# AshishKumar4/FlaxDiff

Hardware: AMD Instinct MI355X
Metric: train images/sec/node (64x64 uncond EDM UNet, bs=256) (higher is better)
Workload: dtype bf16; 1 GPU; model=unet_64px_[64,128,256,512]_res2_heads4, global_batch=256, resolution=64, parallelism=dp1, schedule=EDM + KarrasPredictionTransform(sigma_data=0.5)

## Files before the change

flaxdiff_amd/models/common.py:

```python
from __future__ import annotations

import math
from typing import Callable, Optional

import torch
import torch.nn as nn
import torch.nn.functional as F

from .. import ops


_TRUNC_STD_CORRECTION = 0.87962566103423978


def variance_scaling_(tensor: torch.Tensor, fan_in: int, fan_out: int,
                      scale: float = 1.0, mode: str = "fan_in") -> torch.Tensor:
    if mode == "fan_in":
        denom = max(1, fan_in)
    elif mode == "fan_out":
        denom = max(1, fan_out)
    else:
        denom = max(1.0, (fan_in + fan_out) / 2)
    std = math.sqrt(max(scale, 1e-10) / denom) / _TRUNC_STD_CORRECTION
    with torch.no_grad():
        tensor.normal_(0.0, std)
        tensor.clamp_(-2 * std, 2 * std)
    return tensor


class _ShadowCast(torch.autograd.Function):

    @staticmethod
    def forward(ctx, p):
        return p._shadow_bf16

    @staticmethod
    def backward(ctx, dy):
        return dy.float()


def _cast(p: Optional[torch.Tensor], dtype) -> Optional[torch.Tensor]:
    if p is None:
        return None
    if p.dtype == dtype:
        return p
    if dtype == torch.bfloat16 and getattr(p, "_shadow_bf16", None) is not None:
        return _ShadowCast.apply(p)
    return p.to(dtype)



class Dense(nn.Module):
    def __init__(self, in_features: int, out_features: int, use_bias: bool = True,
                 kernel_scale: float = 1.0, zero_init: bool = False):
        super().__init__()
        self.in_features = in_features
        self.out_features = out_features
        w = torch.empty(in_features, out_features)
        if zero_init:
            nn.init.zeros_(w)
        else:
            variance_scaling_(w, in_features, out_features, scale=kernel_scale)
        self.weight = nn.Parameter(w)
        self.bias = nn.Parameter(torch.zeros(out_features)) if use_bias else None

    def forward(self, x: torch.Tensor, add: torch.Tensor = None) -> torch.Tensor:
        if x.is_cuda and x.dtype == torch.bfloat16:
            return ops.dense(x, self.weight, self.bias, add=add)
        return ops.dense(x, _cast(self.weight, x.dtype),
                         _cast(self.bias, x.dtype), add=add)



class GroupNorm(nn.Module):

    def __init__(self, num_groups: int, num_channels: int, eps: float = 1e-5):
        super().__init__()
        assert num_channels % num_groups == 0, (num_groups, num_channels)
        self.num_groups = num_groups
        self.eps = eps
        self.weight = nn.Parameter(torch.ones(num_channels))
        self.bias = nn.Parameter(torch.zeros(num_channels))

    def forward(self, x: torch.Tensor, silu: bool = False) -> torch.Tensor:
        if x.is_cuda:
            return ops.group_norm(x, self.num_groups, self.weight, self.bias,
                                  self.eps, silu)
        return ops.group_norm(x, self.num_groups, _cast(self.weight, x.dtype),
                              _cast(self.bias, x.dtype), self.eps, silu)


class RMSNorm(nn.Module):
    def __init__(self, dim: int, eps: float = 1e-5):
        super().__init__()
        self.eps = eps
        self.weight = nn.Parameter(torch.ones(dim))

    def forward(self, x: torch.Tensor) -> torch.Tensor:
        if x.is_cuda:
            return ops.rms_norm(x, self.weight, self.eps)
        return ops.rms_norm(x, _cast(self.weight, x.dtype), self.eps)



class TimeEmbedding(nn.Module):

    def __init__(self, features: int, max_positions: int = 10000):
        super().__init__()
        self.features = features
        self.max_positions = max_positions

    def forward(self, t: torch.Tensor) -> torch.Tensor:
        return ops.sinusoidal_time_embedding(t, self.features, self.max_positions)


class FourierEmbedding(nn.Module):

    def __init__(self, features: int, scale: float = 16.0):
        super().__init__()
        g = torch.Generator().manual_seed(42)
        freqs = torch.randn(features // 2, generator=g) * scale
        self.register_buffer("freqs", freqs, persistent=True)

    def forward(self, t: torch.Tensor) -> torch.Tensor:
        return ops.fourier_time_embedding(t, self.freqs)


class TimeProjection(nn.Module):

    def __init__(self, in_features: int, features: int):
        super().__init__()
        self.dense1 = Dense(in_features, features)
        self.dense2 = Dense(features, features)

    def forward(self, x: torch.Tensor) -> torch.Tensor:
        x = F.gelu(self.dense1(x))
        x = F.gelu(self.dense2(x))
        return x



class Conv(nn.Module):

    def __init__(self, in_features: int, features: int, kernel_size=(3, 3),
                 strides=(1, 1), use_bias: bool = True):
        super().__init__()
        kh, kw = kernel_size if isinstance(kernel_size, (tuple, list)) \
            else (kernel_size, kernel_size)
        self.stride = strides[0] if isinstance(strides, (tuple, list)) else strides
        w = torch.empty(kh, kw, in_features, features)
        variance_scaling_(w, kh * kw * in_features, kh * kw * features)
        self.weight = nn.Parameter(w)
        self.bias = nn.Parameter(torch.zeros(features)) if use_bias else None

    def forward(self, x: torch.Tensor, add: torch.Tensor = None,
                badd: torch.Tensor = None) -> torch.Tensor:
        if x.is_cuda and x.dtype == torch.bfloat16:
            return ops.conv2d(x, self.weight, self.bias, stride=self.stride,
                              add=add, badd=badd)
        return ops.conv2d(x, _cast(self.weight, x.dtype), _cast(self.bias, x.dtype),
                          stride=self.stride, add=add, badd=badd)


class ConvTranspose(nn.Module):
    def __init__(self, in_features: int, features: int, kernel_size=(3, 3), strides=(2, 2)):
        super().__init__()
        kh, kw = kernel_size
        self.stride = strides[0]
        w = torch.empty(kh, kw, in_features, features)
        variance_scaling_(w, kh * kw * in_features, kh * kw * features)
        self.weight = nn.Parameter(w)
        self.bias = nn.Parameter(torch.zeros(features))

    def forward(self, x):
        return ops.conv2d_transpose(x, _cast(self.weight, x.dtype),
                                    _cast(self.bias, x.dtype), stride=self.stride)


class SeparableConv(nn.Module):

    def __init__(self, in_features: int, features: int, kernel_size=(3, 3),
                 strides=(1, 1), use_bias: bool = False):
        super().__init__()
        kh, kw = kernel_size
        self.stride = strides[0] if isinstance(strides, (tuple, list)) else strides
        dw = torch.empty(kh, kw, in_features, 1)
        variance_scaling_(dw, kh * kw, kh * kw)
        self.depthwise = nn.Parameter(dw)
        pw = torch.empty(1, 1, in_features, features)
        variance_scaling_(pw, in_features, features)
        self.pointwise = nn.Parameter(pw)
        self.bias = nn.Parameter(torch.zeros(features)) if use_bias else None

    def forward(self, x):
        x = ops.depthwise_conv2d(x, _cast(self.depthwise, x.dtype), None, self.stride)
        return ops.conv2d(x, _cast(self.pointwise, x.dtype), _cast(self.bias, x.dtype), 1)


class WeightStandardizedConv(nn.Module):

    def __init__(self, in_features: int, features: int, kernel_size=(3, 3), strides=(1, 1)):
        super().__init__()
        kh, kw = kernel_size
        self.stride = strides[0] if isinstance(strides, (tuple, list)) else strides
        w = torch.empty(kh, kw, in_features, features)
        variance_scaling_(w, kh * kw * in_features, kh * kw * features)
        self.weight = nn.Parameter(w)
        self.bias = nn.Parameter(torch.zeros(features))

    def forward(self, x):
        w = self.weight
        eps = 1e-5 if x.dtype == torch.float32 else 1e-3
        mean = w.mean(dim=(0, 1, 2), keepdim=True)
        var = w.var(dim=(0, 1, 2), unbiased=False, keepdim=True)
        w = (w - mean) / torch.sqrt(var + eps)
        return ops.conv2d(x, _cast(w, x.dtype), _cast(self.bias, x.dtype), self.stride)


def ConvLayer(conv_type: str, in_features: int, features: int, kernel_size=(3, 3),
              strides=(1, 1)) -> nn.Module:
    if conv_type == "conv":
        return Conv(in_features, features, kernel_size, strides)
    if conv_type == "w_conv":
        return WeightStandardizedConv(in_features, features, kernel_size, strides)
    if conv_type == "separable":
        return SeparableConv(in_features, features, kernel_size, strides)
    if conv_type == "conv_transpose":
        return ConvTranspose(in_features, features, kernel_size, strides)
    raise ValueError(f"unknown conv_type {conv_type}")


class PixelShuffle(nn.Module):

    def __init__(self, scale: int):
        super().__init__()
        self.scale = scale

    def forward(self, x):
        B, H, W, C = x.shape
        s = self.scale
        c = C // (s * s)
        x = x.reshape(B, H, W, s, s, c)
        x = x.permute(0, 1, 3, 2, 4, 5)
        return x.reshape(B, H * s, W * s, c)


class Upsample(nn.Module):

    def __init__(self, in_features: int, features: int, scale: int = 2,
                 activation: Callable = F.silu):
        super().__init__()
        assert scale == 2
        self.conv = Conv(in_features, features, (3, 3), (1, 1))

    def forward(self, x, residual=None):
        if x.is_cuda and x.dtype == torch.bfloat16:
            out = ops.conv2d_upsample2x(x, self.conv.weight, self.conv.bias)
        else:
            out = self.conv(ops.nearest_upsample_2x(x))
        if residual is not None:
            out = ops.cat_channels(out, residual)
        return out


class Downsample(nn.Module):

    def __init__(self, in_features: int, features: int, scale: int = 2,
                 activation: Callable = F.silu):
        super().__init__()
        assert scale == 2
        self.conv = Conv(in_features, features, (3, 3), (2, 2))

    def forward(self, x, residual=None):
        out = self.conv(x)
        if residual is not None:
            if residual.shape[1] > out.shape[1]:
                residual = ops.avg_pool_2x(residual)
            out = ops.cat_channels(out, residual)
        return out



class ResidualBlock(nn.Module):

    def __init__(self, conv_type: str, in_features: int, features: int,
                 temb_features: int, kernel_size=(3, 3), strides=(1, 1),
                 activation: Callable = F.silu, norm_groups: int = 8,
                 norm_epsilon: float = 1e-4):
        super().__init__()
        self.features = features
        self.activation = activation
        self._fused_silu = activation in (F.silu, torch.nn.functional.silu)
        if norm_groups > 0:
            self.norm1 = GroupNorm(norm_groups, in_features, eps=norm_epsilon)
            self.norm2 = GroupNorm(norm_groups, features, eps=norm_epsilon)
        else:
            self.norm1 = RMSNorm(in_features, eps=norm_epsilon)
            self.norm2 = RMSNorm(features, eps=norm_epsilon)
        self.conv1 = ConvLayer(conv_type, in_features, features, kernel_size, strides)
        self.temb_projection = Dense(temb_features, features)
        self.conv2 = ConvLayer(conv_type, features, features, kernel_size, strides)
        self.residual_conv = (ConvLayer(conv_type, in_features, features, (1, 1), (1, 1))
                              if in_features != features else None)

    def _norm_act(self, norm, x):
        if isinstance(norm, GroupNorm) and self._fused_silu:
            return norm(x, silu=True)
        return self.activation(norm(x))

    def forward(self, x: torch.Tensor, temb: torch.Tensor,
                textemb: torch.Tensor = None, extra_features: torch.Tensor = None):
        residual = x
        out = self._norm_act(self.norm1, x)
        t = self.temb_projection(temb.to(out.dtype))
        if isinstance(self.conv1, Conv):
            out = self.conv1(out, badd=t)
        else:
            out = self.conv1(out) + t[:, None, None, :]

        out = self._norm_act(self.norm2, out)
        if self.residual_conv is not None:
            residual = self.residual_conv(residual)
        if isinstance(self.conv2, Conv) and residual.shape[-1] == self.features:
            out = self.conv2(out, add=residual)
        else:
            out = self.conv2(out) + residual

        if extra_features is not None:
            out = ops.cat_channels(out, extra_features)
        return out


def l2norm(t: torch.Tensor, dim=1, eps=1e-6):
    return t / torch.clamp(t.norm(p=2, dim=dim, keepdim=True), min=eps)
```

flaxdiff_amd/ops/__init__.py:

```python
from __future__ import annotations

import os
import weakref
from typing import Optional

import torch

from . import reference

_EXT = None
_EXT_ERR: Optional[str] = None


def _load_ext():
    global _EXT, _EXT_ERR
    if _EXT is not None or _EXT_ERR is not None:
        return _EXT
    try:
        from .hip import build as hip_build
        _EXT = hip_build.load_extension()
    except Exception as e:
        _EXT_ERR = f"{type(e).__name__}: {e}"
        _EXT = None
    return _EXT


def hip_available() -> bool:
    return _load_ext() is not None


def _require_ext():
    ext = _load_ext()
    if ext is None:
        raise RuntimeError(
            "flaxdiff_amd HIP extension is not available on a GPU tensor path "
            f"(build error: {_EXT_ERR}). Run __graft_entry__.build() / "
            "python -m flaxdiff_amd.ops.hip.build first — the GPU path never "
            "silently falls back to stock torch ops.")
    return ext


_FORCE_TORCH = os.environ.get("FLAXDIFF_FORCE_TORCH_OPS", "0") == "1"
_GEMM_LIB = os.environ.get("FD_GEMM_LIB", "0") == "1"


def _use_hip(x: torch.Tensor) -> bool:
    return x.is_cuda and not _FORCE_TORCH



_GRAD_HOOK_OWNERS: "weakref.WeakSet" = weakref.WeakSet()


def register_grad_hook_owner(owner) -> None:
    _GRAD_HOOK_OWNERS.add(owner)


def _sink_kinds() -> str:
    v = os.environ.get("FD_GRAD_SINK", "1")
    if v == "0":
        return ""
    return "wbgr" if v == "all" else "bgr"


def grad_sinks_active() -> bool:
    if not _sink_kinds():
        return False
    return not any(o.hooks_live for o in _GRAD_HOOK_OWNERS)


def _grad_sink(p: Optional[torch.Tensor], kind: str) -> Optional[torch.Tensor]:
    if p is None or kind not in _sink_kinds():
        return None
    sink = getattr(p, "_grad_sink", None)
    if sink is None or sink.dtype != torch.float32 or not grad_sinks_active():
        return None
    owner = getattr(p, "_grad_sink_owner", None)
    g = (p if owner is None else owner).grad
    if g is None or g.data_ptr() != sink.data_ptr() \
            or g.numel() != sink.numel() or not sink.is_contiguous():
        return None
    return sink



class _GroupNormSiLUFn(torch.autograd.Function):
    @staticmethod
    def forward(ctx, x, gamma, beta, groups, eps, silu):
        ext = _require_ext()
        y, mean, rstd = ext.gn_silu_fwd(x, gamma, beta, groups, eps, silu)
        ctx.save_for_backward(x, gamma, mean, rstd)
        ctx.groups = groups
        ctx.silu = silu
        ctx.has_beta = beta is not None
        ctx.beta = beta
        ctx.gamma_param = gamma
        return y

    @staticmethod
    def backward(ctx, dy):
        x, gamma, mean, rstd = ctx.saved_tensors
        ext = _require_ext()
        beta = ctx.beta if ctx.has_beta else torch.zeros_like(gamma)
        if ctx.has_beta and ctx.needs_input_grad[1] and ctx.needs_input_grad[2]:
            sg, sb = _grad_sink(ctx.gamma_param, "g"), _grad_sink(ctx.beta, "g")
            if sg is not None and sb is not None:
                (dx,) = ext.gn_silu_bwd(dy.contiguous(), x, gamma, beta, mean,
                                        rstd, ctx.groups, ctx.silu, sg, sb)
                return dx, None, None, None, None, None
        dx, dgamma, dbeta = ext.gn_silu_bwd(dy.contiguous(), x, gamma, beta,
                                            mean, rstd, ctx.groups, ctx.silu)
        return dx, dgamma, (dbeta if ctx.has_beta else None), None, None, None


def group_norm(x: torch.Tensor, groups: int, gamma: torch.Tensor,
               beta: torch.Tensor, eps: float = 1e-5, silu: bool = False) -> torch.Tensor:
    if _use_hip(x):
        return _GroupNormSiLUFn.apply(x.contiguous(), gamma, beta, groups, eps, silu)
    return reference.group_norm_nhwc(x, groups, gamma, beta, eps, silu)



class _RMSNormFn(torch.autograd.Function):
    @staticmethod
    def forward(ctx, x, gamma, eps):
        ext = _require_ext()
        y, rrms = ext.rms_norm_fwd(x, gamma, eps)
        ctx.save_for_backward(x, gamma, rrms)
        ctx.gamma_param = gamma
        return y

    @staticmethod
    def backward(ctx, dy):
        x, gamma, rrms = ctx.saved_tensors
        ext = _require_ext()
        sink = _grad_sink(ctx.gamma_param, "r") if ctx.needs_input_grad[1] else None
        if sink is not None:
            (dx,) = ext.rms_norm_bwd(dy.contiguous(), x, gamma, rrms, sink)
            return dx, None, None
        dx, dgamma = ext.rms_norm_bwd(dy.contiguous(), x, gamma, rrms)
        return dx, dgamma, None


def rms_norm(x: torch.Tensor, gamma: torch.Tensor, eps: float = 1e-5) -> torch.Tensor:
    if _use_hip(x):
        return _RMSNormFn.apply(x.contiguous(), gamma, eps)
    return reference.rms_norm(x, gamma, eps)



def _conv2d_wgrad_gemms(dy: torch.Tensor, x: torch.Tensor, kh: int, kw: int,
                        stride: int) -> torch.Tensor:
    B, H, W, Ci = x.shape
    _, OH, OW, Co = dy.shape
    pt = max((OH - 1) * stride + kh - H, 0) // 2
    pl = max((OW - 1) * stride + kw - W, 0) // 2
    dw = torch.zeros(kh, kw, Ci, Co, dtype=torch.float32, device=x.device)
    for r in range(kh):
        oh_lo = max(0, -((pt - r) // -stride))
        oh_hi = min(OH - 1, (H - 1 - r + pt) // stride)
        if oh_hi < oh_lo:
            continue
        ih_lo = oh_lo * stride + r - pt
        noh = oh_hi - oh_lo + 1
        for s in range(kw):
            ow_lo = max(0, -((pl - s) // -stride))
            ow_hi = min(OW - 1, (W - 1 - s + pl) // stride)
            if ow_hi < ow_lo:
                continue
            iw_lo = ow_lo * stride + s - pl
            now = ow_hi - ow_lo + 1
            x_sub = x[:, ih_lo:ih_lo + (noh - 1) * stride + 1:stride,
                      iw_lo:iw_lo + (now - 1) * stride + 1:stride, :]
            dy_sub = dy[:, oh_lo:oh_hi + 1, ow_lo:ow_hi + 1, :]
            a = x_sub.reshape(-1, Ci)
            b = dy_sub.reshape(-1, Co)
            dw[r, s] += (a.transpose(0, 1) @ b).float()
    return dw


def _kernel_view(p: torch.Tensor) -> torch.Tensor:
    if p.dtype == torch.bfloat16:
        return p
    sh = getattr(p, "_shadow_bf16", None)
    if sh is not None:
        return sh
    return p.to(torch.bfloat16)


def _kernel_view_t(p: torch.Tensor) -> torch.Tensor:
    t = getattr(p, "_shadow_bf16_t", None)
    if t is not None:
        return t
    return _kernel_view(p).t().contiguous()


def transpose_shadows(src_flat, dst_flat, tiles):
    _require_ext().transpose_shadows(src_flat, dst_flat, tiles)


def _routable_param(p: Optional[torch.Tensor]) -> bool:
    return p is None or p.dtype == torch.bfloat16 or \
        getattr(p, "_shadow_bf16", None) is not None


class _Conv2dFn(torch.autograd.Function):
    @staticmethod
    def forward(ctx, x, w, b, stride, add, badd):
        ext = _require_ext()
        wk = _kernel_view(w)
        y = ext.conv2d_fwd(x, wk, b if b is not None else torch.Tensor(),
                           stride,
                           add if add is not None else torch.Tensor(),
                           badd if badd is not None else torch.Tensor())
        ctx.save_for_backward(x, wk)
        ctx.stride = stride
        ctx.has_bias = b is not None
        ctx.has_add = add is not None
        ctx.has_badd = badd is not None
        ctx.w_dtype = w.dtype
        ctx.b_dtype = b.dtype if b is not None else None
        ctx.w_param, ctx.b_param = w, b
        return y

    @staticmethod
    def backward(ctx, dy):
        x, wk = ctx.saved_tensors
        ext = _require_ext()
        dy = dy.contiguous()
        dx = ext.conv2d_dgrad(dy, wk, ctx.stride, x.shape[1], x.shape[2]) \
            if ctx.needs_input_grad[0] else None
        dw = db = None
        b_param = ctx.b_param if ctx.has_bias and ctx.needs_input_grad[2] \
            else None
        if ctx.needs_input_grad[1]:
            dw, db = _wgrad(ext, dy, x, wk.shape[0], wk.shape[1], ctx.stride,
                            ctx.w_param, ctx.w_dtype, b_param, ctx.b_dtype)
        elif ctx.has_bias:
            db = _bias_grad(dy, b_param, ctx.b_dtype)
        dadd = dy if ctx.has_add else None
        dbadd = None
        if ctx.has_badd:
            B = dy.shape[0]
            dbadd = dy.reshape(B, -1, dy.shape[-1]).sum(1)
        return dx, dw, db, None, dadd, dbadd


class _DenseFn(torch.autograd.Function):

    @staticmethod
    def forward(ctx, x2d, w2d, b, add):
        wk = _kernel_view(w2d)
        if not _GEMM_LIB and x2d.shape[1] % 64 == 0:
            ext = _require_ext()
            bf = b if b is not None else torch.Tensor()
            if bf.numel() and bf.dtype != torch.float32:
                bf = bf.float()
            y = ext.gemm_nt(x2d, _kernel_view_t(w2d), bf,
                            add if add is not None else torch.Tensor())
        else:
            y = torch.matmul(x2d, wk)
            if b is not None:
                y = y + _kernel_view(b)
            if add is not None:
                y = y + add
        ctx.save_for_backward(x2d, wk)
        ctx.has_bias = b is not None
        ctx.has_add = add is not None
        ctx.w_dtype = w2d.dtype
        ctx.b_dtype = b.dtype if b is not None else None
        ctx.w_param, ctx.b_param = w2d, b
        return y

    @staticmethod
    def backward(ctx, dy):
        x2d, wk = ctx.saved_tensors
        dy = dy.contiguous()
        ext = _require_ext()
        if ctx.needs_input_grad[0]:
            if not _GEMM_LIB and dy.shape[1] % 64 == 0:
                dx = ext.gemm_dx(dy, wk)
            else:
                dx = torch.matmul(dy, wk.t())
        else:
            dx = None
        dw = db = None
        b_param = ctx.b_param if ctx.has_bias and ctx.needs_input_grad[2] \
            else None
        if ctx.needs_input_grad[1]:
            M = x2d.shape[0]
            dw, db = _wgrad(ext, dy.view(M, 1, 1, dy.shape[1]),
                            x2d.view(M, 1, 1, x2d.shape[1]), 1, 1, 1,
                            ctx.w_param, ctx.w_dtype, b_param, ctx.b_dtype)
            if dw is not None:
                dw = dw.view(x2d.shape[1], dy.shape[1])
        elif ctx.has_bias:
            db = _bias_grad(dy, b_param, ctx.b_dtype)
        dadd = dy if ctx.has_add else None
        return dx, dw, db, dadd


def dense(x: torch.Tensor, w: torch.Tensor, b: Optional[torch.Tensor] = None,
          add: Optional[torch.Tensor] = None) -> torch.Tensor:
    if _use_hip(x) and x.dtype == torch.bfloat16 and _routable_param(w) \
            and _routable_param(b):
        lead = x.shape[:-1]
        add2 = None
        if add is not None and add.dtype == torch.bfloat16:
            add2 = add.reshape(-1, w.shape[1]).contiguous()
        y = _DenseFn.apply(x.reshape(-1, x.shape[-1]).contiguous(), w, b, add2)
        y = y.reshape(*lead, w.shape[1])
        if add is not None and add2 is None:
            y = y + add
        return y
    if w.dtype != x.dtype:
        w = w.to(x.dtype)
    y = torch.matmul(x, w)
    if b is not None:
        y = y + b.to(y.dtype)
    if add is not None:
        y = y + add.to(y.dtype)
    return y


class _WL2LossFn(torch.autograd.Function):

    @staticmethod
    def forward(ctx, pred, target, wb):
        ctx.save_for_backward(pred, target, wb)
        return _require_ext().wl2_loss_fwd(pred, target, wb)

    @staticmethod
    def backward(ctx, go):
        pred, target, wb = ctx.saved_tensors
        dpred = _require_ext().wl2_loss_bwd(pred, target, wb,
                                            go.reshape(1).float())
        return dpred, None, None


def weighted_l2_loss(pred: torch.Tensor, target: torch.Tensor,
                     weights: torch.Tensor) -> torch.Tensor:
    if _use_hip(pred) and pred.dtype == torch.bfloat16 \
            and target.dtype == torch.bfloat16:
        wb = weights.reshape(weights.shape[0]).float().contiguous()
        return _WL2LossFn.apply(pred.contiguous(), target.contiguous(), wb)
    return (0.5 * (pred.float() - target.float()) ** 2
            * weights.to(torch.float32)).mean()


class _ConvUp2xFn(torch.autograd.Function):

    @staticmethod
    def forward(ctx, x, w, b):
        ext = _require_ext()
        wk = _kernel_view(w)
        y = ext.conv2d_fwd_up2x(x, wk, b if b is not None else torch.Tensor())
        if y is None or y.numel() == 0:
            raise _ConvUpIneligibleError
        ctx.save_for_backward(x, wk)
        ctx.has_bias = b is not None
        ctx.w_dtype = w.dtype
        ctx.b_dtype = b.dtype if b is not None else None
        ctx.w_param, ctx.b_param = w, b
        return y

    @staticmethod
    def backward(ctx, dy):
        x, wk = ctx.saved_tensors
        ext = _require_ext()
        dy = dy.contiguous()
        H2, W2 = x.shape[1] * 2, x.shape[2] * 2
        dx = db = dw = None
        b_param = ctx.b_param if ctx.has_bias and ctx.needs_input_grad[2] \
            else None
        if ctx.needs_input_grad[0]:
            dx_up = ext.conv2d_dgrad(dy, wk, 1, H2, W2)
            dx = ext.upsample2x_bwd(dx_up)
        if ctx.needs_input_grad[1]:
            x_up = ext.upsample2x_fwd(x)
            dw, db = _wgrad(ext, dy, x_up, 3, 3, 1, ctx.w_param, ctx.w_dtype,
                            b_param, ctx.b_dtype)
        elif ctx.has_bias:
            db = _bias_grad(dy, b_param, ctx.b_dtype)
        return dx, dw, db


class _ConvUpIneligibleError(Exception):
    pass


def conv2d_upsample2x(x: torch.Tensor, w: torch.Tensor,
                      b: Optional[torch.Tensor] = None) -> torch.Tensor:
    if _use_hip(x) and x.dtype == torch.bfloat16 and _routable_param(w) \
            and w.shape[0] == 3 and w.shape[1] == 3:
        try:
            return _ConvUp2xFn.apply(
                x.contiguous(), w.contiguous(),
                b.contiguous() if b is not None else None)
        except _ConvUpIneligibleError:
            pass
    return conv2d(nearest_upsample_2x(x), w, b, stride=1)


class _GEGLUFn(torch.autograd.Function):

    @staticmethod
    def forward(ctx, h):
        ctx.save_for_backward(h)
        return _require_ext().geglu_fwd(h)

    @staticmethod
    def backward(ctx, dy):
        (h,) = ctx.saved_tensors
        return _require_ext().geglu_bwd(dy.contiguous(), h)


def geglu(h: torch.Tensor) -> torch.Tensor:
    if _use_hip(h) and h.dtype == torch.bfloat16 and h.shape[-1] % 16 == 0:
        return _GEGLUFn.apply(h.contiguous())
    a, b = h.chunk(2, dim=-1)
    return a * torch.nn.functional.gelu(b)


class _Cat2Fn(torch.autograd.Function):

    @staticmethod
    def forward(ctx, a, b):
        ctx.ca = a.shape[-1]
        ctx.cb = b.shape[-1]
        return _require_ext().cat2_lastdim(a, b)

    @staticmethod
    def backward(ctx, dy):
        da, db = _require_ext().split2_lastdim(dy.contiguous(), ctx.ca, ctx.cb)
        return da, db


def cat_channels(a: torch.Tensor, b: torch.Tensor) -> torch.Tensor:
    if _use_hip(a) and a.dtype == torch.bfloat16 and b.dtype == torch.bfloat16 \
            and (a.shape[-1] + b.shape[-1]) % 8 == 0:
        return _Cat2Fn.apply(a.contiguous(), b.contiguous())
    return torch.cat([a, b], dim=-1)


def _wgrad(ext, dy, x, kh, kw, stride, w_param, w_dtype,
           b_param=None, b_dtype=None):
    want_db = b_dtype is not None
    w_sink = _grad_sink(w_param, "w") if w_dtype == torch.float32 else None
    b_sink = _grad_sink(b_param, "b") if b_dtype == torch.float32 else None
    dw, db, folded = ext.conv2d_wgrad(dy, x, kh, kw, stride, w_sink,
                                      want_db, b_sink)
    if dw is not None and w_dtype != torch.float32:
        dw = dw.to(w_dtype)
    if want_db and not folded:
        db = _bias_grad(dy, b_param, b_dtype)
    elif db is not None and b_dtype != torch.float32:
        db = db.to(b_dtype)
    return dw, db


def _bias_grad(dy: torch.Tensor, b_param: Optional[torch.Tensor] = None,
               b_dtype=torch.float32) -> Optional[torch.Tensor]:
    d2 = dy.reshape(-1, dy.shape[-1])
    C = d2.shape[1]
    if d2.is_cuda and d2.dtype == torch.bfloat16 and C % 8 == 0 and C <= 2048:
        sink = _grad_sink(b_param, "b") if b_dtype == torch.float32 else None
        db = _require_ext().colsum(d2.contiguous(), sink)
        if sink is not None:
            return None
    else:
        db = d2.float().sum(0)
    return db if b_dtype == torch.float32 else db.to(b_dtype)


def conv2d(x: torch.Tensor, w: torch.Tensor, b: Optional[torch.Tensor] = None,
           stride: int = 1, add: Optional[torch.Tensor] = None,
           badd: Optional[torch.Tensor] = None) -> torch.Tensor:
    kh, kw = w.shape[0], w.shape[1]
    if kh == 1 and kw == 1 and stride == 1:
        w2 = w.reshape(w.shape[2], w.shape[3])
        sh = getattr(w, "_shadow_bf16", None)
        if sh is not None and w.dtype != torch.bfloat16:
            w2._shadow_bf16 = sh.reshape(w.shape[2], w.shape[3])
            sht = getattr(w, "_shadow_bf16_t", None)
            if sht is not None:
                w2._shadow_bf16_t = sht
            sink = getattr(w, "_grad_sink", None)
            if sink is not None:
                w2._grad_sink = sink.reshape(w.shape[2], w.shape[3])
                w2._grad_sink_owner = w
        y = dense(x.reshape(-1, w.shape[2]), w2, b)
        y = y.reshape(*x.shape[:-1], w.shape[3])
        if badd is not None:
            y = y + badd[:, None, None, :].to(y.dtype)
        return y if add is None else y + add
    if _use_hip(x) and x.dtype == torch.bfloat16 and _routable_param(w):
        if add is not None and add.dtype != torch.bfloat16:
            add_in, add_out = None, add
        else:
            add_in, add_out = add, None
        if badd is not None and badd.dtype != torch.bfloat16:
            badd_in, badd_out = None, badd
        else:
            badd_in, badd_out = badd, None
        out = _Conv2dFn.apply(
            x.contiguous(), w.contiguous(),
            b.contiguous() if b is not None else None, stride,
            add_in.contiguous() if add_in is not None else None,
            badd_in.contiguous() if badd_in is not None else None)
        if badd_out is not None:
            out = out + badd_out[:, None, None, :].to(out.dtype)
        if add_out is not None:
            out = out + add_out
        return out
    if w.dtype != x.dtype:
        w = w.to(x.dtype)
    if b is not None and b.dtype != x.dtype:
        b = b.to(x.dtype)
    y = reference.conv2d_nhwc(x, w, b, stride=stride, padding="same")
    if badd is not None:
        y = y + badd[:, None, None, :].to(y.dtype)
    return y if add is None else y + add


class _ConvTransposeFn(torch.autograd.Function):

    @staticmethod
    def forward(ctx, x, wf, stride):
        ext = _require_ext()
        H2 = x.shape[1] * stride
        W2 = x.shape[2] * stride
        y = ext.conv2d_dgrad(x, wf, stride, H2, W2)
        ctx.save_for_backward(x, wf)
        ctx.stride = stride
        return y

    @staticmethod
    def backward(ctx, dout):
        x, wf = ctx.saved_tensors
        ext = _require_ext()
        dout = dout.contiguous()
        dx = ext.conv2d_fwd(dout, wf, torch.Tensor(), ctx.stride,
                            torch.Tensor(), torch.Tensor()) \
            if ctx.needs_input_grad[0] else None
        dwf = None
        if ctx.needs_input_grad[1]:
            dwf = ext.conv2d_wgrad(x, dout, wf.shape[0], wf.shape[1],
                                   ctx.stride)[0].to(wf.dtype)
        return dx, dwf, None


def conv2d_transpose(x: torch.Tensor, w: torch.Tensor, b: Optional[torch.Tensor] = None,
                     stride: int = 2) -> torch.Tensor:
    kh, kw = w.shape[0], w.shape[1]
    if _use_hip(x) and stride == 2 and kh == 3 and kw == 3:
        wf = w.permute(0, 1, 3, 2).contiguous()
        out = _ConvTransposeFn.apply(x.contiguous(), wf, stride)
        if b is not None:
            out = out + b
        return out
    return reference.conv2d_transpose_nhwc(x, w, b, stride)


class _DepthwiseConvFn(torch.autograd.Function):

    @staticmethod
    def forward(ctx, x, w, stride, dilation):
        ext = _require_ext()
        y = ext.dwconv_fwd(x, w, None, stride, dilation)
        ctx.save_for_backward(x, w)
        ctx.stride = stride
        ctx.dilation = dilation
        return y

    @staticmethod
    def backward(ctx, dy):
        x, w = ctx.saved_tensors
        ext = _require_ext()
        dy = dy.contiguous()
        dx = ext.dwconv_dgrad(dy, w, x.shape[1], x.shape[2],
                              ctx.stride, ctx.dilation)
        dw = ext.dwconv_wgrad(dy, x, ctx.stride, ctx.dilation)
        return dx, dw.to(w.dtype), None, None


def depthwise_conv2d(x: torch.Tensor, w: torch.Tensor, b: Optional[torch.Tensor] = None,
                     stride: int = 1, dilation: int = 1) -> torch.Tensor:
    if (_use_hip(x) and x.dtype == torch.bfloat16 and b is None
            and w.shape[0] == 3 and w.shape[1] == 3 and x.shape[-1] % 8 == 0):
        w3 = w.reshape(3, 3, -1).contiguous()
        return _DepthwiseConvFn.apply(x, w3, stride, dilation)
    return reference.depthwise_conv2d_nhwc(x, w, b, stride, dilation)



class _AttentionFn(torch.autograd.Function):
    @staticmethod
    def forward(ctx, q, k, v, scale):
        ext = _require_ext()
        o, lse = ext.attn_fwd(q, k, v, scale)
        ctx.save_for_backward(q, k, v, lse)
        ctx.scale = scale
        return o

    @staticmethod
    def backward(ctx, do):
        q, k, v, lse = ctx.saved_tensors
        scale = ctx.scale
        use_v1 = os.environ.get("FD_ATTN_BWD_V1")
        dmax = 32 if use_v1 else 64
        if k.shape[2] <= 128 and q.shape[3] <= dmax:
            ext = _require_ext()
            fn = ext.attn_bwd_smallkv if use_v1 else ext.attn_bwd_smallkv_v2
            dq, dk, dv = fn(q, k, v, do.contiguous(), lse, scale)
            return dq, dk, dv, None
        qf, kf, vf, dof = q.float(), k.float(), v.float(), do.float()
        s = torch.einsum("bhqd,bhkd->bhqk", qf, kf) * scale
        p = torch.exp(s - lse.unsqueeze(-1))
        dv = torch.einsum("bhqk,bhqd->bhkd", p, dof)
        dp = torch.einsum("bhqd,bhkd->bhqk", dof, vf)
        dsum = (dp * p).sum(-1, keepdim=True)
        ds = (dp - dsum) * p * scale
        dq = torch.einsum("bhqk,bhkd->bhqd", ds, kf)
        dk = torch.einsum("bhqk,bhqd->bhkd", ds, qf)
        return dq.to(q.dtype), dk.to(k.dtype), dv.to(v.dtype), None


def attention(q: torch.Tensor, k: torch.Tensor, v: torch.Tensor,
              scale: Optional[float] = None) -> torch.Tensor:
    if scale is None:
        scale = q.shape[-1] ** -0.5
    if _use_hip(q):
        D = q.shape[-1]
        if D % 8 == 0 and D <= 128:
            return _AttentionFn.apply(q.contiguous(), k.contiguous(),
                                      v.contiguous(), scale)
    return reference.attention(q, k, v, scale)



def forward_diffusion(x0, eps, signal_rate, noise_rate):
    if _use_hip(x0):
        ext = _require_ext()
        return ext.fwd_diffusion(x0, eps, signal_rate.reshape(-1).float().contiguous(),
                                 noise_rate.reshape(-1).float().contiguous())
    return reference.forward_diffusion(x0, eps, signal_rate, noise_rate)


def nearest_upsample_2x(x: torch.Tensor) -> torch.Tensor:
    if _use_hip(x):
        ext = _require_ext()
        return _Upsample2xFn.apply(x.contiguous())
    return reference.nearest_upsample_2x_nhwc(x)


class _Upsample2xFn(torch.autograd.Function):
    @staticmethod
    def forward(ctx, x):
        ext = _require_ext()
        return ext.upsample2x_fwd(x)

    @staticmethod
    def backward(ctx, dy):
        ext = _require_ext()
        return ext.upsample2x_bwd(dy.contiguous())


def avg_pool_2x(x: torch.Tensor) -> torch.Tensor:
    return reference.avg_pool_2x_nhwc(x)


def sinusoidal_time_embedding(t: torch.Tensor, features: int,
                              max_positions: int = 10000) -> torch.Tensor:
    if _use_hip(t):
        ext = _require_ext()
        return ext.time_embed(t, torch.Tensor(), features, float(max_positions))
    return reference.sinusoidal_time_embedding(t, features, max_positions)


def fourier_time_embedding(t: torch.Tensor, freqs: torch.Tensor) -> torch.Tensor:
    if _use_hip(t):
        ext = _require_ext()
        return ext.time_embed(t, freqs, freqs.numel() * 2, 0.0)
    return reference.fourier_time_embedding(t, freqs)



class _S5ScanFn(torch.autograd.Function):

    @staticmethod
    def forward(ctx, a_ri, bu_ri):
        ext = _require_ext()
        x = ext.s5_scan_fwd(a_ri.contiguous(), bu_ri.contiguous())
        ctx.save_for_backward(a_ri, x)
        return x

    @staticmethod
    def backward(ctx, dx):
        a_ri, x = ctx.saved_tensors
        ext = _require_ext()
        dbu, dap = ext.s5_scan_bwd(a_ri.contiguous(), x, dx.contiguous())
        return dap.sum(dim=0), dbu


def s5_scan(a: torch.Tensor, bu: torch.Tensor) -> torch.Tensor:
    if bu.is_cuda and not _FORCE_TORCH:
        a_ri = torch.view_as_real(a.contiguous()).float()
        bu_ri = torch.view_as_real(bu.contiguous()).float()
        x = _S5ScanFn.apply(a_ri, bu_ri)
        return torch.view_as_complex(x)
    from ..models.ssm_dit import associative_scan_diag
    return associative_scan_diag(a.reshape(1, 1, -1).expand_as(bu), bu)


def fused_adamw_ema(params_f32, grads, exp_avg, exp_avg_sq, ema_f32, params_bf16,
                    *, lr, beta1, beta2, eps, weight_decay, step, ema_decay,
                    grad_scale: float = 1.0, scale_dev=None, skip_ctr=None,
                    step_dev=None):
    ext = _require_ext()
    ext.fused_adamw_ema(params_f32, grads, exp_avg, exp_avg_sq, ema_f32,
                        params_bf16 if params_bf16 is not None else torch.Tensor(),
                        lr, beta1, beta2, eps, weight_decay, step, ema_decay,
                        grad_scale, scale_dev, skip_ctr, step_dev)
```

flaxdiff_amd/ops/hip/attention.hip:

```cpp
#include <torch/extension.h>
#include <ATen/hip/HIPContext.h>
#include "common.h"

typedef __bf16 bf16v8 __attribute__((ext_vector_type(8)));

#define ATT_TILE 64
#define NTH 256

union ABF8 { bf16v8 v; ushort u[8]; uint4 q; };

template <int QI, int NCH>
__global__ __launch_bounds__(NTH, 2)
void attn_fwd_kernel(const ushort* __restrict__ Q,
                     const ushort* __restrict__ K,
                     const ushort* __restrict__ V,
                     ushort* __restrict__ O,
                     float* __restrict__ LSE,
                     const int Sq, const int Skv, const int D,
                     const float scale) {
    constexpr int Dp = NCH * 32;
    constexpr int NDF = Dp / 16;
    constexpr int KROW = Dp + 8;
    constexpr int VROW = ATT_TILE + 8;
    constexpr int PROW = ATT_TILE + 8;
    extern __shared__ __attribute__((aligned(16))) char smem[];
    ushort* Kl = reinterpret_cast<ushort*>(smem);
    ushort* Vl = Kl + ATT_TILE * KROW;
    ushort* Pl = Vl + Dp * VROW;

    const int bh = blockIdx.y;
    const long q_blk = (long)blockIdx.x * (QI * 64);
    const int tid = threadIdx.x;
    const int lane = tid & 63;
    const int wid = tid >> 6;
    const int l15 = lane & 15;
    const int l4 = lane >> 4;

    const ushort* Qb = Q + (long)bh * Sq * D;
    const ushort* Kb = K + (long)bh * Skv * D;
    const ushort* Vb = V + (long)bh * Skv * D;

    ABF8 qf[QI][NCH];
    #pragma unroll
    for (int qi = 0; qi < QI; ++qi) {
        const long qrow = q_blk + (qi * 4 + wid) * 16 + l15;
        #pragma unroll
        for (int c = 0; c < NCH; ++c) {
            qf[qi][c].q = make_uint4(0, 0, 0, 0);
            const int d0 = c * 32 + l4 * 8;
            if (qrow < Sq && d0 < D) {
                if (d0 + 8 <= D) {
                    qf[qi][c].q = *reinterpret_cast<const uint4*>(Qb + qrow * D + d0);
                } else {
                    for (int j = 0; j < 8 && d0 + j < D; ++j)
                        qf[qi][c].u[j] = Qb[qrow * D + d0 + j];
                }
            }
        }
    }

    float m_run[QI][4], l_run[QI][4];
    f32x4 oacc[QI][NDF] = {};
    #pragma unroll
    for (int qi = 0; qi < QI; ++qi)
        #pragma unroll
        for (int r = 0; r < 4; ++r) { m_run[qi][r] = -1e30f; l_run[qi][r] = 0.f; }

    const int ntiles = (Skv + ATT_TILE - 1) / ATT_TILE;
    for (int t = 0; t < ntiles; ++t) {
        const int kv0 = t * ATT_TILE;
        __syncthreads();
        for (int lin = tid; lin < ATT_TILE * (Dp / 8); lin += NTH) {
            const int kv = lin / (Dp / 8);
            const int d0 = (lin % (Dp / 8)) * 8;
            ABF8 kval; kval.q = make_uint4(0, 0, 0, 0);
            ABF8 vval; vval.q = make_uint4(0, 0, 0, 0);
            if (kv0 + kv < Skv && d0 < D) {
                const long src = (long)(kv0 + kv) * D + d0;
                if (d0 + 8 <= D) {
                    kval.q = *reinterpret_cast<const uint4*>(Kb + src);
                    vval.q = *reinterpret_cast<const uint4*>(Vb + src);
                } else {
                    for (int j = 0; j < 8 && d0 + j < D; ++j) {
                        kval.u[j] = Kb[src + j];
                        vval.u[j] = Vb[src + j];
                    }
                }
            }
            *reinterpret_cast<uint4*>(Kl + kv * KROW + d0) = kval.q;
            #pragma unroll
            for (int j = 0; j < 8; ++j)
                Vl[(d0 + j) * VROW + kv] = vval.u[j];
        }
        __syncthreads();


        #pragma unroll
        for (int qi = 0; qi < QI; ++qi) {
            f32x4 sfr[4] = {};
            #pragma unroll
            for (int f = 0; f < 4; ++f) {
                #pragma unroll
                for (int c = 0; c < NCH; ++c) {
                    bf16v8 bb = reinterpret_cast<const ABF8*>(
                        Kl + (f * 16 + l15) * KROW + c * 32 + l4 * 8)->v;
                    sfr[f] = __builtin_amdgcn_mfma_f32_16x16x32_bf16(
                        qf[qi][c].v, bb, sfr[f], 0, 0, 0);
                }
            }

            float tmax[4] = {-1e30f, -1e30f, -1e30f, -1e30f};
            float sv[4][4];
            #pragma unroll
            for (int f = 0; f < 4; ++f) {
                const int kv = kv0 + f * 16 + l15;
                #pragma unroll
                for (int r = 0; r < 4; ++r) {
                    float s = sfr[f][r] * scale;
                    if (kv >= Skv) s = -1e30f;
                    sv[f][r] = s;
                    tmax[r] = fmaxf(tmax[r], s);
                }
            }
            #pragma unroll
            for (int r = 0; r < 4; ++r) {
                #pragma unroll
                for (int off = 1; off < 16; off <<= 1)
                    tmax[r] = fmaxf(tmax[r], __shfl_xor(tmax[r], off, 64));
            }

            float alpha[4];
            #pragma unroll
            for (int r = 0; r < 4; ++r) {
                const float mn = fmaxf(m_run[qi][r], tmax[r]);
                alpha[r] = expf(m_run[qi][r] - mn);
                m_run[qi][r] = mn;
                l_run[qi][r] *= alpha[r];
            }
            #pragma unroll
            for (int f = 0; f < NDF; ++f) {
                #pragma unroll
                for (int r = 0; r < 4; ++r) oacc[qi][f][r] *= alpha[r];
            }

            float rsum[4] = {0.f, 0.f, 0.f, 0.f};
            #pragma unroll
            for (int f = 0; f < 4; ++f) {
                #pragma unroll
                for (int r = 0; r < 4; ++r) {
                    const float p = expf(sv[f][r] - m_run[qi][r]);
                    rsum[r] += p;
                    Pl[(wid * 16 + l4 * 4 + r) * PROW + f * 16 + l15] = f2bf(p);
                }
            }
            #pragma unroll
            for (int r = 0; r < 4; ++r) {
                #pragma unroll
                for (int off = 1; off < 16; off <<= 1)
                    rsum[r] += __shfl_xor(rsum[r], off, 64);
                l_run[qi][r] += rsum[r];
            }
            __syncthreads();

            #pragma unroll
            for (int kc = 0; kc < ATT_TILE / 32; ++kc) {
                bf16v8 pa = reinterpret_cast<const ABF8*>(
                    Pl + (wid * 16 + l15) * PROW + kc * 32 + l4 * 8)->v;
                #pragma unroll
                for (int f = 0; f < NDF; ++f) {
                    bf16v8 vb = reinterpret_cast<const ABF8*>(
                        Vl + (f * 16 + l15) * VROW + kc * 32 + l4 * 8)->v;
                    oacc[qi][f] = __builtin_amdgcn_mfma_f32_16x16x32_bf16(
                        pa, vb, oacc[qi][f], 0, 0, 0);
                }
            }
        }
    }

    ushort* Ob = O + (long)bh * Sq * D;
    float* Lb = LSE + (long)bh * Sq;
    #pragma unroll
    for (int qi = 0; qi < QI; ++qi) {
        float inv_l[4];
        #pragma unroll
        for (int r = 0; r < 4; ++r)
            inv_l[r] = (l_run[qi][r] > 0.f) ? 1.f / l_run[qi][r] : 0.f;
        const long qbase = q_blk + (qi * 4 + wid) * 16;
        #pragma unroll
        for (int f = 0; f < NDF; ++f) {
            const int d = f * 16 + l15;
            if (d >= D) continue;
            #pragma unroll
            for (int r = 0; r < 4; ++r) {
                const long qrow = qbase + l4 * 4 + r;
                if (qrow < Sq)
                    Ob[qrow * D + d] = f2bf(oacc[qi][f][r] * inv_l[r]);
            }
        }
        if (l15 == 0) {
            #pragma unroll
            for (int r = 0; r < 4; ++r) {
                const long qrow = qbase + l4 * 4 + r;
                if (qrow < Sq)
                    Lb[qrow] = m_run[qi][r] + logf(fmaxf(l_run[qi][r], 1e-30f));
            }
        }
    }
}

std::vector<torch::Tensor> attn_fwd(torch::Tensor q, torch::Tensor k,
                                    torch::Tensor v, double scale) {
    FD_FLUSH_STALE();
    TORCH_CHECK(q.is_cuda() && q.is_contiguous() && q.dim() == 4);
    TORCH_CHECK(q.scalar_type() == at::kBFloat16, "attn kernel is bf16");
    const int B = q.size(0), H = q.size(1), Sq = q.size(2), D = q.size(3);
    const int Skv = k.size(2);
    TORCH_CHECK(D <= 128 && D % 8 == 0, "attn: D must be <=128, mult of 8; got ", D);

    auto o = torch::empty_like(q);
    auto lse = torch::empty({B, H, Sq}, q.options().dtype(at::kFloat));

    const int Dp = (D + 31) & ~31;
    const int nch = Dp / 32;
    const int qi = (nch == 1) ? (D <= 16 ? 8 : 4) : (nch == 2 ? 2 : 1);
    const size_t smem = ((size_t)ATT_TILE * (Dp + 8)
                         + (size_t)Dp * (ATT_TILE + 8)
                         + 4ul * 16 * (ATT_TILE + 8))
                        * sizeof(ushort);
    dim3 grid((Sq + qi * 64 - 1) / (qi * 64), B * H);
    auto stream = at::hip::getCurrentHIPStream();
    #define ATT_LAUNCH(QI_, NCH_) \
        hipLaunchKernelGGL((attn_fwd_kernel<QI_, NCH_>), grid, dim3(NTH), smem, \
                           stream, (const ushort*)q.data_ptr(), \
                           (const ushort*)k.data_ptr(), \
                           (const ushort*)v.data_ptr(), (ushort*)o.data_ptr(), \
                           lse.data_ptr<float>(), Sq, Skv, D, (float)scale)
    if (nch == 1 && qi == 8) ATT_LAUNCH(8, 1);
    else if (nch == 1) ATT_LAUNCH(4, 1);
    else if (nch == 2) ATT_LAUNCH(2, 2);
    else if (nch == 3) ATT_LAUNCH(1, 3);
    else ATT_LAUNCH(1, 4);
    #undef ATT_LAUNCH
    FD_CHECK_LAUNCH();
    return {o, lse};
}
```

flaxdiff_amd/ops/hip/attention_bwd_v2.hip:

```cpp
#include <torch/extension.h>
#include <ATen/hip/HIPContext.h>
#include "common.h"

typedef __bf16 bf16v8b __attribute__((ext_vector_type(8)));
typedef __attribute__((__vector_size__(4 * sizeof(__bf16)))) __bf16 bf16x4b;

#define AB2_MAXNTH 512

union BBF8 { bf16v8b v; ushort u[8]; uint4 q; ushort4 h4[2]; };

__device__ __forceinline__ bf16x4b ab2_tr(const ushort* p) {
    return __builtin_amdgcn_ds_read_tr16_b64_v4bf16(
        (__attribute__((address_space(3))) bf16x4b*)p);
}

__device__ __forceinline__ int ab2_dfrag_row(int r, int half) {
    return (r & 3) + 8 * (r >> 2) + 4 * half;
}

template <int DP, int NJF, int NW = ((NJF == 4 || DP >= 64) ? 4 : 8)>
__global__ __launch_bounds__(NW * 64, 1)
void attn_bwd_v2_kernel(const ushort* __restrict__ Q,
                        const ushort* __restrict__ K,
                        const ushort* __restrict__ V,
                        const ushort* __restrict__ dO,
                        const float* __restrict__ LSE,
                        ushort* __restrict__ dQ,
                        ushort* __restrict__ dKo,
                        ushort* __restrict__ dVo,
                        const int Sq, const int Skv, const int D,
                        const float scale) {
    constexpr int NDP = DP / 16;
    constexpr int NDH = DP > 32 ? DP / 32 : 1;
    constexpr int NQI = NDP < 2 ? 2 : NDP;
    constexpr int QROWS = 36;
    constexpr int PQS = QROWS * 16;
    constexpr int JT = NJF * 32;
    constexpr int JTP = JT + 4;
    constexpr int PPS = JTP * 16;

    extern __shared__ __attribute__((aligned(16))) ushort ab2m[];
    ushort* Kp = ab2m;
    ushort* Vp = Kp + NDP * PPS;
    ushort* wbase = Vp + NDP * PPS;
    const int tid = threadIdx.x;
    const int lane = tid & 63;
    const int wid = tid >> 6;
    const int l31 = lane & 31;
    const int half = lane >> 5;
    const int WSZ = 2 * 2 * PPS + 2 * NQI * PQS;
    ushort* Pt = wbase + wid * WSZ;
    ushort* dSt = Pt + 2 * PPS;
    ushort* Qp = dSt + 2 * PPS;
    ushort* dOp = Qp + NQI * PQS;

    const int bh = blockIdx.x;
    const ushort* Qb = Q + (long)bh * Sq * D;
    const ushort* Kb = K + (long)bh * Skv * D;
    const ushort* Vb = V + (long)bh * Skv * D;
    const ushort* dOb = dO + (long)bh * Sq * D;
    const float* lse_b = LSE + (long)bh * Sq;

    for (int i = tid; i < NDP * PPS; i += NW * 64) {
        const int p = i / PPS;
        const int j = (i % PPS) >> 4;
        const int d = p * 16 + (i & 15);
        ushort kv = 0, vv = 0;
        if (j < Skv && d < D) {
            kv = Kb[(long)j * D + d];
            vv = Vb[(long)j * D + d];
        }
        Kp[i] = kv;
        Vp[i] = vv;
    }
    for (int i = tid; i < NQI * PQS; i += NW * 64) {
        Qp[(i / PQS) * PQS + (i % PQS)] = 0;
        dOp[(i / PQS) * PQS + (i % PQS)] = 0;
    }
    __syncthreads();

    f32x16 dk_acc[NJF][NDH] = {}, dv_acc[NJF][NDH] = {};
    const int nq_iters = (Sq + 32 * NW - 1) / (32 * NW);

    for (int it = 0; it < nq_iters; ++it) {
        const long q0 = (long)it * 32 * NW + wid * 32;
        const bool qvalid = q0 < Sq;

        BBF8 qf[NDP], dof[NDP];
        #pragma unroll
        for (int c = 0; c < NDP; ++c) {
            qf[c].q = make_uint4(0, 0, 0, 0);
            dof[c].q = make_uint4(0, 0, 0, 0);
            const long qrow = q0 + l31;
            const int d0 = c * 16 + half * 8;
            if (qvalid && qrow < Sq && d0 < D) {
                if (d0 + 8 <= D) {
                    qf[c].q = *reinterpret_cast<const uint4*>(Qb + qrow * D + d0);
                    dof[c].q = *reinterpret_cast<const uint4*>(dOb + qrow * D + d0);
                } else {
                    for (int t = 0; t < 8 && d0 + t < D; ++t) {
                        qf[c].u[t] = Qb[qrow * D + d0 + t];
                        dof[c].u[t] = dOb[qrow * D + d0 + t];
                    }
                }
            }
            ushort* qd = Qp + c * PQS + l31 * 16 + half * 8;
            ushort* od = dOp + c * PQS + l31 * 16 + half * 8;
            *reinterpret_cast<uint2*>(qd) = make_uint2(qf[c].q.x, qf[c].q.y);
            *reinterpret_cast<uint2*>(qd + 4) = make_uint2(qf[c].q.z, qf[c].q.w);
            *reinterpret_cast<uint2*>(od) = make_uint2(dof[c].q.x, dof[c].q.y);
            *reinterpret_cast<uint2*>(od + 4) = make_uint2(dof[c].q.z, dof[c].q.w);
        }

        float lse_r[16];
        #pragma unroll
        for (int r = 0; r < 16; ++r) {
            long qi = q0 + ab2_dfrag_row(r, half);
            qi = qi < Sq ? qi : Sq - 1;
            qi = qi < 0 ? 0 : qi;
            lse_r[r] = lse_b[qi];
        }

        float dsum[16] = {};
        #pragma unroll
            for (int fc = 0; fc < NJF; ++fc) {
            f32x16 s_acc = {}, dp_acc = {};
            #pragma unroll
            for (int c = 0; c < NDP; ++c) {
                const bf16v8b kfr = reinterpret_cast<const BBF8*>(
                    Kp + c * PPS + (fc * 32 + l31) * 16 + half * 8)->v;
                const bf16v8b vfr = reinterpret_cast<const BBF8*>(
                    Vp + c * PPS + (fc * 32 + l31) * 16 + half * 8)->v;
                s_acc = __builtin_amdgcn_mfma_f32_32x32x16_bf16(qf[c].v, kfr, s_acc, 0, 0, 0);
                dp_acc = __builtin_amdgcn_mfma_f32_32x32x16_bf16(dof[c].v, vfr, dp_acc, 0, 0, 0);
            }
            const int j = fc * 32 + l31;
            const bool jok = j < Skv;
            #pragma unroll
            for (int g = 0; g < 4; ++g) {
                ushort4 pv, dv4;
                #pragma unroll
                for (int t = 0; t < 4; ++t) {
                    const int r = g * 4 + t;
                    const int qr = ab2_dfrag_row(r, half);
                    const bool ok = qvalid & jok & (q0 + qr < Sq);
                    const float p = ok ? __expf(s_acc[r] * scale - lse_r[r]) : 0.f;
                    const float dp = ok ? dp_acc[r] : 0.f;
                    dsum[r] += p * dp;
                    reinterpret_cast<ushort*>(&pv)[t] = f2bf(p);
                    reinterpret_cast<ushort*>(&dv4)[t] = f2bf(dp);
                }
                const int qpos = g * 8 + half * 4;
                const int qp = qpos >> 4, qoff = qpos & 15;
                *reinterpret_cast<ushort4*>(Pt + qp * PPS + j * 16 + qoff) = pv;
                *reinterpret_cast<ushort4*>(dSt + qp * PPS + j * 16 + qoff) = dv4;
            }
        }
        #pragma unroll
        for (int r = 0; r < 16; ++r) {
            float v = dsum[r];
            #pragma unroll
            for (int off = 16; off > 0; off >>= 1)
                v += __shfl_xor(v, off, 32);
            dsum[r] = v;
        }

        #pragma unroll
            for (int fc = 0; fc < NJF; ++fc) {
            const int j = fc * 32 + l31;
            #pragma unroll
            for (int g = 0; g < 4; ++g) {
                const int qpos = g * 8 + half * 4;
                const int qp = qpos >> 4, qoff = qpos & 15;
                const ushort4 pv = *reinterpret_cast<const ushort4*>(
                    Pt + qp * PPS + j * 16 + qoff);
                ushort4 dv4 = *reinterpret_cast<const ushort4*>(
                    dSt + qp * PPS + j * 16 + qoff);
                #pragma unroll
                for (int t = 0; t < 4; ++t) {
                    const int r = g * 4 + t;
                    const float p = bf2f(reinterpret_cast<const ushort*>(&pv)[t]);
                    const float dp = bf2f(reinterpret_cast<const ushort*>(&dv4)[t]);
                    reinterpret_cast<ushort*>(&dv4)[t] =
                        f2bf((dp - dsum[r]) * p * scale);
                }
                *reinterpret_cast<ushort4*>(dSt + qp * PPS + j * 16 + qoff) = dv4;
            }
        }
        __builtin_amdgcn_wave_barrier();
        asm volatile("s_waitcnt lgkmcnt(0)");

        const int trq0 = ((lane >> 4) & 1) * PQS + ((lane >> 5) << 3) * 16
                       + (lane & 15) * 4;
        #pragma unroll
            for (int fc = 0; fc < NJF; ++fc) {
            #pragma unroll
            for (int c = 0; c < 2; ++c) {
                const int k0 = c * 16 + half * 8;
                const bf16v8b pa = reinterpret_cast<const BBF8*>(
                    Pt + (k0 >> 4) * PPS + (fc * 32 + l31) * 16 + (k0 & 15))->v;
                const bf16v8b dsa = reinterpret_cast<const BBF8*>(
                    dSt + (k0 >> 4) * PPS + (fc * 32 + l31) * 16 + (k0 & 15))->v;
                #pragma unroll
                for (int dh = 0; dh < NDH; ++dh) {
                    const int trq = trq0 + dh * 2 * PQS;
                    bf16x4b o1 = ab2_tr(dOp + trq + c * 16 * 16);
                    bf16x4b o2 = ab2_tr(dOp + trq + c * 16 * 16 + 64);
                    bf16x4b q1 = ab2_tr(Qp + trq + c * 16 * 16);
                    bf16x4b q2 = ab2_tr(Qp + trq + c * 16 * 16 + 64);
                    BBF8 obf, qbf;
                    obf.h4[0] = *reinterpret_cast<ushort4*>(&o1);
                    obf.h4[1] = *reinterpret_cast<ushort4*>(&o2);
                    qbf.h4[0] = *reinterpret_cast<ushort4*>(&q1);
                    qbf.h4[1] = *reinterpret_cast<ushort4*>(&q2);
                    dv_acc[fc][dh] = __builtin_amdgcn_mfma_f32_32x32x16_bf16(pa, obf.v, dv_acc[fc][dh], 0, 0, 0);
                    dk_acc[fc][dh] = __builtin_amdgcn_mfma_f32_32x32x16_bf16(dsa, qbf.v, dk_acc[fc][dh], 0, 0, 0);
                }
            }
        }

        if (qvalid) {
            f32x16 dq_acc[NDH] = {};
            const int trp = ((lane >> 4) & 1) * PPS + (lane & 15) * 4;
            #pragma unroll
            for (int c = 0; c < JT / 16; ++c) {
                const int mrow = (c * 16 + (half << 3)) * 16;
                bf16x4b a1 = ab2_tr(dSt + trp + mrow);
                bf16x4b a2 = ab2_tr(dSt + trp + mrow + 64);
                BBF8 af;
                af.h4[0] = *reinterpret_cast<ushort4*>(&a1);
                af.h4[1] = *reinterpret_cast<ushort4*>(&a2);
                #pragma unroll
                for (int dh = 0; dh < NDH; ++dh) {
                    const int trk = (dh * 2 + ((lane >> 4) & 1)) * PPS
                                  + (lane & 15) * 4;
                    bf16x4b b1 = ab2_tr(Kp + trk + mrow);
                    bf16x4b b2 = ab2_tr(Kp + trk + mrow + 64);
                    BBF8 bf;
                    bf.h4[0] = *reinterpret_cast<ushort4*>(&b1);
                    bf.h4[1] = *reinterpret_cast<ushort4*>(&b2);
                    dq_acc[dh] = __builtin_amdgcn_mfma_f32_32x32x16_bf16(af.v, bf.v, dq_acc[dh], 0, 0, 0);
                }
            }
            __builtin_amdgcn_wave_barrier();
            asm volatile("s_waitcnt lgkmcnt(0)");
            ushort* dqs = dOp;
            #pragma unroll
            for (int dh = 0; dh < NDH; ++dh) {
                const int d = dh * 32 + l31;
                #pragma unroll
                for (int g = 0; g < 4; ++g) {
                    ushort4 payload;
                    #pragma unroll
                    for (int t = 0; t < 4; ++t)
                        reinterpret_cast<ushort*>(&payload)[t] =
                            f2bf(dq_acc[dh][g * 4 + t]);
                    const int qpos = g * 8 + half * 4;
                    if (d < DP)
                        *reinterpret_cast<ushort4*>(dqs + d * QROWS + qpos) = payload;
                }
            }
            __builtin_amdgcn_wave_barrier();
            asm volatile("s_waitcnt lgkmcnt(0)");
            const int qr = l31;
            #pragma unroll
            for (int pass = 0; pass < DP / 16; ++pass) {
                const int d0 = (half + 2 * pass) * 8;
                if (q0 + qr < Sq && d0 < D) {
                    BBF8 outv;
                    #pragma unroll
                    for (int t = 0; t < 8; ++t)
                        outv.u[t] = (d0 + t < D) ? dqs[(d0 + t) * QROWS + qr] : (ushort)0;
                    if (d0 + 8 <= D) {
                        *reinterpret_cast<uint4*>(dQ + ((long)bh * Sq + q0 + qr) * D + d0) = outv.q;
                    } else {
                        for (int t = 0; t < 8 && d0 + t < D; ++t)
                            dQ[((long)bh * Sq + q0 + qr) * D + d0 + t] = outv.u[t];
                    }
                }
            }
        }
    }

    float* dkf = reinterpret_cast<float*>(ab2m);
    float* dvf = dkf + JT * DP;
    __syncthreads();
    for (int i = tid; i < JT * DP; i += NW * 64) {
        dkf[i] = 0.f;
        dvf[i] = 0.f;
    }
    __syncthreads();
    #pragma unroll
    for (int fc = 0; fc < NJF; ++fc) {
        #pragma unroll
        for (int dh = 0; dh < NDH; ++dh) {
            const int d = dh * 32 + l31;
            #pragma unroll
            for (int r = 0; r < 16; ++r) {
                const int j = fc * 32 + ab2_dfrag_row(r, half);
                if (d < DP) {
                    atomicAdd(dkf + j * DP + d, dk_acc[fc][dh][r]);
                    atomicAdd(dvf + j * DP + d, dv_acc[fc][dh][r]);
                }
            }
        }
    }
    __syncthreads();
    for (int i = tid; i < Skv * D; i += NW * 64) {
        const int j = i / D, d = i - (i / D) * D;
        dKo[((long)bh * Skv + j) * D + d] = f2bf(dkf[j * DP + d]);
        dVo[((long)bh * Skv + j) * D + d] = f2bf(dvf[j * DP + d]);
    }
}

std::vector<torch::Tensor> attn_bwd_smallkv_v2(torch::Tensor q, torch::Tensor k,
                                               torch::Tensor v, torch::Tensor dout,
                                               torch::Tensor lse, double scale) {
    FD_FLUSH_STALE();
    TORCH_CHECK(q.is_cuda() && q.is_contiguous() && k.is_contiguous() &&
                v.is_contiguous() && dout.is_contiguous());
    TORCH_CHECK(q.scalar_type() == at::kBFloat16);
    const int B = q.size(0), H = q.size(1), Sq = q.size(2), D = q.size(3);
    const int Skv = k.size(2);
    TORCH_CHECK(Skv <= 128 && D <= 64);
    auto lse_c = lse.contiguous();
    const int JT = ((Skv + 31) / 32) * 32;
    const int JTP = JT + 4;

    auto dq = torch::empty_like(q);
    auto dk = torch::empty_like(k);
    auto dv = torch::empty_like(v);

    auto stream = at::hip::getCurrentHIPStream();
    const int nwaves = (JT / 32 == 4 || D > 32) ? 4 : 8;
    auto launch = [&](auto kern, int DPv) {
        const int NDP = DPv / 16;
        const size_t smem_fwd = (2 * (size_t)NDP * JTP * 16
            + (size_t)nwaves * (2 * 2 * (size_t)JTP * 16 + 2 * 2 * 36 * 16))
            * sizeof(ushort);
        const size_t smem_acc = 2 * (size_t)JT * DPv * sizeof(float);
        const size_t smem = std::max(smem_fwd, smem_acc);
        static bool attr_set[16] = {};
        int slot = (DPv == 16 ? 0 : 8) + JT / 32;
        if (!attr_set[slot]) {
            hipFuncSetAttribute((const void*)kern,
                                hipFuncAttributeMaxDynamicSharedMemorySize,
                                160 * 1024);
            attr_set[slot] = true;
        }
        hipLaunchKernelGGL(kern, dim3(B * H), dim3(nwaves * 64), smem, stream,
                           (const ushort*)q.data_ptr(), (const ushort*)k.data_ptr(),
                           (const ushort*)v.data_ptr(), (const ushort*)dout.data_ptr(),
                           lse_c.data_ptr<float>(), (ushort*)dq.data_ptr(),
                           (ushort*)dk.data_ptr(), (ushort*)dv.data_ptr(),
                           Sq, Skv, D, (float)scale);
    };
    const int njf = JT / 32;
    if (D <= 16) {
        if (njf == 1) launch(attn_bwd_v2_kernel<16, 1>, 16);
        else if (njf == 2) launch(attn_bwd_v2_kernel<16, 2>, 16);
        else if (njf == 3) launch(attn_bwd_v2_kernel<16, 3>, 16);
        else launch(attn_bwd_v2_kernel<16, 4>, 16);
    } else if (D <= 32) {
        if (njf == 1) launch(attn_bwd_v2_kernel<32, 1>, 32);
        else if (njf == 2) launch(attn_bwd_v2_kernel<32, 2>, 32);
        else if (njf == 3) launch(attn_bwd_v2_kernel<32, 3>, 32);
        else launch(attn_bwd_v2_kernel<32, 4>, 32);
    } else {
        if (njf == 1) launch(attn_bwd_v2_kernel<64, 1>, 64);
        else if (njf == 2) launch(attn_bwd_v2_kernel<64, 2>, 64);
        else if (njf == 3) launch(attn_bwd_v2_kernel<64, 3>, 64);
        else launch(attn_bwd_v2_kernel<64, 4>, 64);
    }
    FD_CHECK_LAUNCH();
    return {dq, dk, dv};
}
```

flaxdiff_amd/ops/hip/bindings.cpp:

```cpp
#include <torch/extension.h>
#include <tuple>
#include <vector>

std::vector<torch::Tensor> gn_silu_fwd(torch::Tensor x, torch::Tensor gamma,
                                       torch::Tensor beta, long groups,
                                       double eps, bool silu);
std::vector<torch::Tensor> gn_silu_bwd(torch::Tensor dy, torch::Tensor x,
                                       torch::Tensor gamma, torch::Tensor beta,
                                       torch::Tensor mean, torch::Tensor rstd,
                                       long groups, bool silu,
                                       c10::optional<torch::Tensor> dgamma_sink,
                                       c10::optional<torch::Tensor> dbeta_sink);
std::vector<torch::Tensor> rms_norm_fwd(torch::Tensor x, torch::Tensor gamma,
                                        double eps);
std::vector<torch::Tensor> rms_norm_bwd(torch::Tensor dy, torch::Tensor x,
                                        torch::Tensor gamma, torch::Tensor rrms,
                                        c10::optional<torch::Tensor> dgamma_sink);
torch::Tensor conv2d_fwd(torch::Tensor x, torch::Tensor w, torch::Tensor bias,
                         long stride, torch::Tensor add, torch::Tensor badd);
torch::Tensor conv2d_fwd_up2x(torch::Tensor x, torch::Tensor w,
                              torch::Tensor bias);
torch::Tensor conv2d_dgrad(torch::Tensor dy, torch::Tensor w, long stride,
                           long H, long W);
std::tuple<torch::Tensor, torch::Tensor, bool>
conv2d_wgrad(torch::Tensor dy, torch::Tensor x, long kh, long kw, long stride,
             c10::optional<torch::Tensor> dw_sink, bool want_db,
             c10::optional<torch::Tensor> db_sink);
torch::Tensor dwconv_fwd(torch::Tensor x, torch::Tensor w,
                         c10::optional<torch::Tensor> bias,
                         int64_t stride, int64_t dilation);
torch::Tensor dwconv_dgrad(torch::Tensor dy, torch::Tensor w,
                           int64_t H, int64_t W, int64_t stride, int64_t dilation);
torch::Tensor dwconv_wgrad(torch::Tensor dy, torch::Tensor x,
                           int64_t stride, int64_t dilation);
std::vector<torch::Tensor> attn_fwd(torch::Tensor q, torch::Tensor k,
                                    torch::Tensor v, double scale);
std::vector<torch::Tensor> attn_bwd_smallkv(torch::Tensor q, torch::Tensor k,
                                            torch::Tensor v, torch::Tensor dout,
                                            torch::Tensor lse, double scale);
std::vector<torch::Tensor> attn_bwd_smallkv_v2(torch::Tensor q, torch::Tensor k,
                                               torch::Tensor v, torch::Tensor dout,
                                               torch::Tensor lse, double scale);
torch::Tensor fwd_diffusion(torch::Tensor x0, torch::Tensor eps,
                            torch::Tensor a, torch::Tensor s);
torch::Tensor upsample2x_fwd(torch::Tensor x);
torch::Tensor time_embed(torch::Tensor t, torch::Tensor freqs, long features,
                         double max_positions);
torch::Tensor upsample2x_bwd(torch::Tensor dy);
torch::Tensor colsum(torch::Tensor x, c10::optional<torch::Tensor> sink);
torch::Tensor cat2_lastdim(torch::Tensor a, torch::Tensor b);
std::vector<torch::Tensor> split2_lastdim(torch::Tensor dy, long Ca, long Cb);
torch::Tensor geglu_fwd(torch::Tensor h);
torch::Tensor geglu_bwd(torch::Tensor dy, torch::Tensor h);
torch::Tensor wl2_loss_fwd(torch::Tensor pred, torch::Tensor target,
                           torch::Tensor wb);
torch::Tensor wl2_loss_bwd(torch::Tensor pred, torch::Tensor target,
                           torch::Tensor wb, torch::Tensor go);
torch::Tensor s5_scan_fwd(torch::Tensor a, torch::Tensor bu);
std::vector<torch::Tensor> s5_scan_bwd(torch::Tensor a, torch::Tensor x,
                                       torch::Tensor dx);
torch::Tensor gemm_fwd(torch::Tensor x, torch::Tensor w, torch::Tensor bias);
torch::Tensor gemm_dx(torch::Tensor dy, torch::Tensor w);
torch::Tensor gemm_nt(torch::Tensor x, torch::Tensor wt, torch::Tensor bias,
                      torch::Tensor add);
void transpose_shadows(torch::Tensor src_flat, torch::Tensor dst_flat,
                       torch::Tensor tiles);
void fused_adamw_ema(torch::Tensor p, torch::Tensor g, torch::Tensor m,
                     torch::Tensor v, torch::Tensor ema, torch::Tensor p_bf16,
                     double lr, double beta1, double beta2, double eps,
                     double weight_decay, long step, double ema_decay,
                     double grad_scale,
                     c10::optional<torch::Tensor> scale_dev,
                     c10::optional<torch::Tensor> skip_ctr,
                     c10::optional<torch::Tensor> step_dev);

PYBIND11_MODULE(TORCH_EXTENSION_NAME, m) {
    m.def("gn_silu_fwd", &gn_silu_fwd, "fused GroupNorm+SiLU forward (NHWC)");
    m.def("gn_silu_bwd", &gn_silu_bwd, "fused GroupNorm+SiLU backward",
          py::arg("dy"), py::arg("x"), py::arg("gamma"), py::arg("beta"),
          py::arg("mean"), py::arg("rstd"), py::arg("groups"), py::arg("silu"),
          py::arg("dgamma_sink") = py::none(), py::arg("dbeta_sink") = py::none());
    m.def("rms_norm_fwd", &rms_norm_fwd, "RMSNorm forward");
    m.def("rms_norm_bwd", &rms_norm_bwd, "RMSNorm backward",
          py::arg("dy"), py::arg("x"), py::arg("gamma"), py::arg("rrms"),
          py::arg("dgamma_sink") = py::none());
    m.def("conv2d_fwd", &conv2d_fwd, "implicit-GEMM NHWC conv forward");
    m.def("conv2d_fwd_up2x", &conv2d_fwd_up2x, "fused nearest-2x upsample + conv forward");
    m.def("conv2d_dgrad", &conv2d_dgrad, "implicit-GEMM NHWC conv dgrad");
    m.def("conv2d_wgrad", &conv2d_wgrad,
          "split-M NHWC conv wgrad (+ folded bias grad): (dw, db, folded)",
          py::arg("dy"), py::arg("x"), py::arg("kh"), py::arg("kw"),
          py::arg("stride"), py::arg("dw_sink") = py::none(),
          py::arg("want_db") = false, py::arg("db_sink") = py::none());
    m.def("dwconv_fwd", &dwconv_fwd, "3x3 depthwise NHWC conv forward");
    m.def("dwconv_dgrad", &dwconv_dgrad, "3x3 depthwise NHWC conv dgrad");
    m.def("dwconv_wgrad", &dwconv_wgrad, "3x3 depthwise NHWC conv wgrad (fp32)");
    m.def("attn_fwd", &attn_fwd, "flash attention forward (bf16, fp32 softmax)");
    m.def("attn_bwd_smallkv", &attn_bwd_smallkv,
          "fused attention backward for Skv<=128, D<=32");
    m.def("attn_bwd_smallkv_v2", &attn_bwd_smallkv_v2,
          "vectorized-LDS attention backward for Skv<=128, D<=32");
    m.def("fwd_diffusion", &fwd_diffusion, "forward-diffusion axpy");
    m.def("upsample2x_fwd", &upsample2x_fwd, "nearest 2x upsample");
    m.def("time_embed", &time_embed, "fused sinusoidal/Fourier time embedding");
    m.def("upsample2x_bwd", &upsample2x_bwd, "nearest 2x upsample backward");
    m.def("colsum", &colsum, "coalesced column sum (bias grads)",
          py::arg("x"), py::arg("sink") = py::none());
    m.def("cat2_lastdim", &cat2_lastdim, "fused last-dim 2-tensor concat");
    m.def("split2_lastdim", &split2_lastdim, "one-pass last-dim split (cat backward)");
    m.def("geglu_fwd", &geglu_fwd, "fused GEGLU forward");
    m.def("geglu_bwd", &geglu_bwd, "fused GEGLU backward");
    m.def("wl2_loss_fwd", &wl2_loss_fwd, "fused weighted L2 loss forward");
    m.def("wl2_loss_bwd", &wl2_loss_bwd, "fused weighted L2 loss backward");
    m.def("s5_scan_fwd", &s5_scan_fwd, "S5 diagonal scan forward");
    m.def("s5_scan_bwd", &s5_scan_bwd, "S5 diagonal scan backward");
    m.def("gemm_fwd", &gemm_fwd, "MFMA bf16 GEMM y = x@w (+bias)");
    m.def("gemm_dx", &gemm_dx, "MFMA bf16 GEMM dx = dy@w^T");
    m.def("gemm_nt", &gemm_nt, "MFMA bf16 GEMM y = x@wt^T (+bias)");
    m.def("transpose_shadows", &transpose_shadows,
          "batched 64x64 bf16 transpose (dense-weight shadow refresh)");
    m.def("fused_adamw_ema", &fused_adamw_ema, "fused AdamW + EMA flat step");
}
```

flaxdiff_amd/ops/hip/common.h:

```cpp
#pragma once

#include <hip/hip_runtime.h>
#include <hip/hip_bf16.h>
#include <hip/hip_fp16.h>
#include <cstdint>

#define FD_WAVE 64

__device__ __forceinline__ float bf2f(ushort u) {
    union { uint32_t i; float f; } c;
    c.i = uint32_t(u) << 16;
    return c.f;
}

__device__ __forceinline__ ushort f2bf(float f) {
    union { float f; uint32_t i; } c;
    c.f = f;
    uint32_t x = c.i;
    uint32_t lsb = (x >> 16) & 1;
    x += 0x7fff + lsb;
    return ushort(x >> 16);
}

typedef ushort ushort8 __attribute__((ext_vector_type(8)));
typedef float float8 __attribute__((ext_vector_type(8)));
typedef short bf16x8 __attribute__((ext_vector_type(8)));
typedef short bf16x4 __attribute__((ext_vector_type(4)));
typedef float f32x4 __attribute__((ext_vector_type(4)));
typedef float f32x16 __attribute__((ext_vector_type(16)));

struct BF16Tag {};
struct F32Tag {};

template <typename T> struct ElemIO;
template <> struct ElemIO<ushort> {
    static __device__ __forceinline__ float ld(const ushort* p) { return bf2f(*p); }
    static __device__ __forceinline__ void st(ushort* p, float v) { *p = f2bf(v); }
};
template <> struct ElemIO<float> {
    static __device__ __forceinline__ float ld(const float* p) { return *p; }
    static __device__ __forceinline__ void st(float* p, float v) { *p = v; }
};

struct FastDiv {
    unsigned long long magic;
    unsigned shift;
    unsigned d;
};

inline FastDiv make_fastdiv(unsigned d) {
    FastDiv f;
    f.d = d;
    unsigned s = 0;
    while ((1ull << s) < d) ++s;
    f.shift = 32 + s;
    f.magic = ((1ull << (32 + s)) + d - 1) / d;
    return f;
}

__device__ __forceinline__ unsigned fd_div(unsigned n, const FastDiv f) {
    return (unsigned)(((unsigned long long)n * f.magic) >> f.shift);
}

__device__ __forceinline__ unsigned fd_mod(unsigned n, unsigned q, const FastDiv f) {
    return n - q * f.d;
}

__device__ __forceinline__ float wave_reduce_sum(float v) {
    #pragma unroll
    for (int off = 32; off > 0; off >>= 1)
        v += __shfl_xor(v, off, FD_WAVE);
    return v;
}

__device__ __forceinline__ float wave_reduce_max(float v) {
    #pragma unroll
    for (int off = 32; off > 0; off >>= 1)
        v = fmaxf(v, __shfl_xor(v, off, FD_WAVE));
    return v;
}

template <int BLOCK>
__device__ __forceinline__ float block_reduce_sum(float v, float* scratch) {
    constexpr int NW = BLOCK / FD_WAVE;
    const int lane = threadIdx.x & (FD_WAVE - 1);
    const int wid = threadIdx.x / FD_WAVE;
    v = wave_reduce_sum(v);
    if (lane == 0) scratch[wid] = v;
    __syncthreads();
    float r = (threadIdx.x < NW) ? scratch[threadIdx.x] : 0.f;
    if (wid == 0) {
        #pragma unroll
        for (int off = NW / 2; off > 0; off >>= 1)
            r += __shfl_xor(r, off, FD_WAVE);
        if (lane == 0) scratch[0] = r;
    }
    __syncthreads();
    float out = scratch[0];
    __syncthreads();
    return out;
}

#define FD_FLUSH_STALE() do { (void)hipGetLastError(); } while (0)
#define FD_CHECK_LAUNCH() do { \
    hipError_t _e = hipGetLastError(); \
    if (_e != hipSuccess) { \
        TORCH_CHECK(false, "HIP kernel launch failed: ", hipGetErrorString(_e)); \
    } } while (0)
```

flaxdiff_amd/ops/hip/gn_silu.hip:

```cpp
#include <torch/extension.h>
#include <ATen/hip/HIPContext.h>
#include "common.h"

template <typename T, bool SILU>
__global__ void gn_silu_fwd_kernel(const T* __restrict__ x,
                                   const float* __restrict__ gamma,
                                   const float* __restrict__ beta,
                                   T* __restrict__ y,
                                   float* __restrict__ mean_out,
                                   float* __restrict__ rstd_out,
                                   int S, int C, int G, float eps) {
    const int b = blockIdx.x / G;
    const int g = blockIdx.x % G;
    const int Cg = C / G;
    const long base = (long)b * S * C + (long)g * Cg;
    const long n = (long)S * Cg;

    __shared__ float scratch[4];

    float s1 = 0.f, s2 = 0.f;
    for (long i = threadIdx.x; i < n; i += blockDim.x) {
        const int s = i / Cg, c = i % Cg;
        const float v = ElemIO<T>::ld(x + base + (long)s * C + c);
        s1 += v; s2 += v * v;
    }
    s1 = block_reduce_sum<256>(s1, scratch);
    s2 = block_reduce_sum<256>(s2, scratch);
    const float mean = s1 / n;
    const float var = fmaxf(s2 / n - mean * mean, 0.f);
    const float rstd = rsqrtf(var + eps);
    if (threadIdx.x == 0) {
        mean_out[blockIdx.x] = mean;
        rstd_out[blockIdx.x] = rstd;
    }

    for (long i = threadIdx.x; i < n; i += blockDim.x) {
        const int s = i / Cg, c = i % Cg;
        const long idx = base + (long)s * C + c;
        const float xn = (ElemIO<T>::ld(x + idx) - mean) * rstd;
        float z = xn * gamma[g * Cg + c] + beta[g * Cg + c];
        if (SILU) z = z / (1.f + expf(-z));
        ElemIO<T>::st(y + idx, z);
    }
}

template <typename T, bool SILU>
__global__ void gn_silu_bwd_kernel(const T* __restrict__ dy,
                                   const T* __restrict__ x,
                                   const float* __restrict__ gamma,
                                   const float* __restrict__ beta,
                                   const float* __restrict__ mean_in,
                                   const float* __restrict__ rstd_in,
                                   T* __restrict__ dx,
                                   float* __restrict__ dgamma,
                                   float* __restrict__ dbeta,
                                   int S, int C, int G) {
    const int b = blockIdx.x / G;
    const int g = blockIdx.x % G;
    const int Cg = C / G;
    const long base = (long)b * S * C + (long)g * Cg;
    const long n = (long)S * Cg;
    const float mean = mean_in[blockIdx.x];
    const float rstd = rstd_in[blockIdx.x];

    extern __shared__ __attribute__((aligned(16))) char smem_raw[];
    float* dg_loc = reinterpret_cast<float*>(smem_raw);
    float* db_loc = dg_loc + Cg;
    float* scratch = db_loc + Cg;
    for (int c = threadIdx.x; c < Cg; c += blockDim.x) {
        dg_loc[c] = 0.f; db_loc[c] = 0.f;
    }
    __syncthreads();

    const int nsub = blockDim.x / Cg;
    const bool active = threadIdx.x < nsub * Cg;
    const int c = threadIdx.x % Cg;
    const int s0 = threadIdx.x / Cg;
    const float gam = gamma[g * Cg + c];
    const float bet = SILU ? beta[g * Cg + c] : 0.f;

    float s1 = 0.f, s2 = 0.f, dg_p = 0.f, db_p = 0.f;
    if (active) {
        for (int s = s0; s < S; s += nsub) {
            const long idx = base + (long)s * C + c;
            const float xn = (ElemIO<T>::ld(x + idx) - mean) * rstd;
            float dz = ElemIO<T>::ld(dy + idx);
            if (SILU) {
                const float z = xn * gam + bet;
                const float sig = 1.f / (1.f + expf(-z));
                dz *= sig * (1.f + z * (1.f - sig));
            }
            dg_p += dz * xn;
            db_p += dz;
            const float dzg = dz * gam;
            s1 += dzg;
            s2 += dzg * xn;
        }
    }
    s1 = block_reduce_sum<256>(s1, scratch);
    s2 = block_reduce_sum<256>(s2, scratch);
    const float inv_n = 1.f / n;

    if (active) {
        for (int s = s0; s < S; s += nsub) {
            const long idx = base + (long)s * C + c;
            const float xn = (ElemIO<T>::ld(x + idx) - mean) * rstd;
            float dz = ElemIO<T>::ld(dy + idx);
            if (SILU) {
                const float z = xn * gam + bet;
                const float sig = 1.f / (1.f + expf(-z));
                dz *= sig * (1.f + z * (1.f - sig));
            }
            ElemIO<T>::st(dx + idx, rstd * (dz * gam - (s1 + xn * s2) * inv_n));
        }
        atomicAdd(dg_loc + c, dg_p);
        atomicAdd(db_loc + c, db_p);
    }

    __syncthreads();
    for (int cc = threadIdx.x; cc < Cg; cc += blockDim.x) {
        atomicAdd(dgamma + g * Cg + cc, dg_loc[cc]);
        atomicAdd(dbeta + g * Cg + cc, db_loc[cc]);
    }
}

union GNV8 { uint4 q; ushort u[8]; };


#define GN3_NTH 256

template <bool SILU>
__global__ void gn3_fwd_stats_kernel(const ushort* __restrict__ x,
                                     float* __restrict__ sums,
                                     const int S, const int C, const int G,
                                     const int Cg, const int chunk_rows,
                                     const FastDiv fdCg) {
    extern __shared__ float sm[];
    const int b = blockIdx.x;
    const int s0 = blockIdx.y * chunk_rows;
    const int s1lim = min(s0 + chunk_rows, S);
    const int tpr = C >> 3;
    const int nsub = GN3_NTH / tpr;
    const bool active = (int)threadIdx.x < nsub * tpr && nsub > 0;
    const int c8 = (threadIdx.x % tpr) * 8;
    const int srow = threadIdx.x / tpr;
    for (int i = threadIdx.x; i < 2 * G; i += GN3_NTH) sm[i] = 0.f;
    __syncthreads();

    float a1 = 0.f, a2 = 0.f;
    if (active) {
        for (int s = s0 + srow; s < s1lim; s += nsub) {
            GNV8 pk;
            pk.q = *reinterpret_cast<const uint4*>(
                x + ((long)b * S + s) * C + c8);
            #pragma unroll
            for (int j = 0; j < 8; ++j) {
                const float v = bf2f(pk.u[j]);
                a1 += v; a2 += v * v;
            }
        }
        const int g = (int)fd_div((unsigned)c8, fdCg);
        atomicAdd(sm + g * 2 + 0, a1);
        atomicAdd(sm + g * 2 + 1, a2);
    }
    __syncthreads();
    for (int i = threadIdx.x; i < 2 * G; i += GN3_NTH)
        if (sm[i] != 0.f) atomicAdd(sums + (long)b * 2 * G + i, sm[i]);
}

template <bool SILU>
__global__ void gn3_fwd_apply_kernel(const ushort* __restrict__ x,
                                     const float* __restrict__ sums,
                                     const float* __restrict__ gamma,
                                     const float* __restrict__ beta,
                                     ushort* __restrict__ y,
                                     float* __restrict__ mean_out,
                                     float* __restrict__ rstd_out,
                                     const int S, const int C, const int G,
                                     const int Cg, const int chunk_rows,
                                     const float eps, const FastDiv fdCg) {
    extern __shared__ float sm[];
    float* mr = sm;
    float* gam = sm + 2 * G;
    float* bet = gam + C;
    const int b = blockIdx.x;
    const int s0 = blockIdx.y * chunk_rows;
    const int s1lim = min(s0 + chunk_rows, S);
    const long base = ((long)b * S + s0) * C;
    const long n = (long)(s1lim - s0) * C;
    const float inv_n = 1.f / ((long)S * Cg);
    for (int g = threadIdx.x; g < G; g += GN3_NTH) {
        const float m = sums[(long)b * 2 * G + g * 2 + 0] * inv_n;
        const float var = fmaxf(sums[(long)b * 2 * G + g * 2 + 1] * inv_n - m * m, 0.f);
        mr[g * 2 + 0] = m;
        mr[g * 2 + 1] = rsqrtf(var + eps);
        if (blockIdx.y == 0) {
            mean_out[(long)b * G + g] = m;
            rstd_out[(long)b * G + g] = mr[g * 2 + 1];
        }
    }
    for (int c = threadIdx.x; c < C; c += GN3_NTH) {
        gam[c] = gamma[c];
        bet[c] = beta[c];
    }
    __syncthreads();

    unsigned cc = (unsigned)((threadIdx.x * 8) % C);
    const unsigned cstep = (unsigned)((GN3_NTH * 8) % C);
    for (long i = (long)threadIdx.x * 8; i < n; i += GN3_NTH * 8) {
        const unsigned c0 = cc;
        cc += cstep; if (cc >= (unsigned)C) cc -= C;
        const int g = (int)fd_div(c0, fdCg);
        const float m = mr[g * 2 + 0], r = mr[g * 2 + 1];
        GNV8 pk, out;
        pk.q = *reinterpret_cast<const uint4*>(x + base + i);
        #pragma unroll
        for (int j = 0; j < 8; ++j) {
            float z = (bf2f(pk.u[j]) - m) * r * gam[c0 + j] + bet[c0 + j];
            if (SILU) z = z / (1.f + __expf(-z));
            out.u[j] = f2bf(z);
        }
        *reinterpret_cast<uint4*>(y + base + i) = out.q;
    }
}

template <bool SILU>
__global__ void gn3_bwd_stats_kernel(const ushort* __restrict__ dy,
                                     const ushort* __restrict__ x,
                                     const float* __restrict__ gamma,
                                     const float* __restrict__ beta,
                                     const float* __restrict__ mean_in,
                                     const float* __restrict__ rstd_in,
                                     float* __restrict__ gsums,
                                     float* __restrict__ dgamma,
                                     float* __restrict__ dbeta,
                                     const int S, const int C, const int G,
                                     const int Cg, const int chunk_rows,
                                     const FastDiv fdCg) {
    extern __shared__ float sm[];
    float* ss = sm;
    float* dgl = ss + 2 * G;
    float* dbl = dgl + C;
    const int b = blockIdx.x;
    const int s0 = blockIdx.y * chunk_rows;
    const int s1lim = min(s0 + chunk_rows, S);
    const int tpr = C >> 3;
    const int nsub = GN3_NTH / tpr;
    const bool active = (int)threadIdx.x < nsub * tpr && nsub > 0;
    const int c8 = (threadIdx.x % tpr) * 8;
    const int srow = threadIdx.x / tpr;
    for (int i = threadIdx.x; i < 2 * G; i += GN3_NTH) ss[i] = 0.f;
    for (int c = threadIdx.x; c < C; c += GN3_NTH) { dgl[c] = 0.f; dbl[c] = 0.f; }
    __syncthreads();

    if (active) {
        const int g = (int)fd_div((unsigned)c8, fdCg);
        const float m = mean_in[(long)b * G + g];
        const float r = rstd_in[(long)b * G + g];
        float g8[8], b8[8], dg8[8] = {}, db8[8] = {};
        #pragma unroll
        for (int j = 0; j < 8; ++j) {
            g8[j] = gamma[c8 + j];
            b8[j] = SILU ? beta[c8 + j] : 0.f;
        }
        float a1 = 0.f, a2 = 0.f;
        for (int s = s0 + srow; s < s1lim; s += nsub) {
            const long idx = ((long)b * S + s) * C + c8;
            GNV8 xv, dv;
            xv.q = *reinterpret_cast<const uint4*>(x + idx);
            dv.q = *reinterpret_cast<const uint4*>(dy + idx);
            #pragma unroll
            for (int j = 0; j < 8; ++j) {
                const float xn = (bf2f(xv.u[j]) - m) * r;
                float dz = bf2f(dv.u[j]);
                if (SILU) {
                    const float z = xn * g8[j] + b8[j];
                    const float sig = 1.f / (1.f + __expf(-z));
                    dz *= sig * (1.f + z * (1.f - sig));
                }
                dg8[j] += dz * xn;
                db8[j] += dz;
                const float dzg = dz * g8[j];
                a1 += dzg;
                a2 += dzg * xn;
            }
        }
        atomicAdd(ss + g * 2 + 0, a1);
        atomicAdd(ss + g * 2 + 1, a2);
        #pragma unroll
        for (int j = 0; j < 8; ++j) {
            atomicAdd(dgl + c8 + j, dg8[j]);
            atomicAdd(dbl + c8 + j, db8[j]);
        }
    }
    __syncthreads();
    for (int i = threadIdx.x; i < 2 * G; i += GN3_NTH)
        if (ss[i] != 0.f) atomicAdd(gsums + (long)b * 2 * G + i, ss[i]);
    for (int c = threadIdx.x; c < C; c += GN3_NTH) {
        if (dgl[c] != 0.f) atomicAdd(dgamma + c, dgl[c]);
        if (dbl[c] != 0.f) atomicAdd(dbeta + c, dbl[c]);
    }
}

template <bool SILU>
__global__ void gn3_bwd_apply_kernel(const ushort* __restrict__ dy,
                                     const ushort* __restrict__ x,
                                     const float* __restrict__ gamma,
                                     const float* __restrict__ beta,
                                     const float* __restrict__ mean_in,
                                     const float* __restrict__ rstd_in,
                                     const float* __restrict__ gsums,
                                     ushort* __restrict__ dx,
                                     const int S, const int C, const int G,
                                     const int Cg, const int chunk_rows,
                                     const FastDiv fdCg) {
    extern __shared__ float sm[];
    float* mrs = sm;
    float* gam = sm + 4 * G;
    float* bet = gam + C;
    const int b = blockIdx.x;
    const int s0 = blockIdx.y * chunk_rows;
    const int s1lim = min(s0 + chunk_rows, S);
    const long base = ((long)b * S + s0) * C;
    const long n = (long)(s1lim - s0) * C;
    for (int g = threadIdx.x; g < G; g += GN3_NTH) {
        mrs[g * 4 + 0] = mean_in[(long)b * G + g];
        mrs[g * 4 + 1] = rstd_in[(long)b * G + g];
        mrs[g * 4 + 2] = gsums[(long)b * 2 * G + g * 2 + 0];
        mrs[g * 4 + 3] = gsums[(long)b * 2 * G + g * 2 + 1];
    }
    for (int c = threadIdx.x; c < C; c += GN3_NTH) {
        gam[c] = gamma[c];
        bet[c] = SILU ? beta[c] : 0.f;
    }
    __syncthreads();
    const float inv_n = 1.f / ((long)S * Cg);

    unsigned cc = (unsigned)((threadIdx.x * 8) % C);
    const unsigned cstep = (unsigned)((GN3_NTH * 8) % C);
    for (long i = (long)threadIdx.x * 8; i < n; i += GN3_NTH * 8) {
        const unsigned c0 = cc;
        cc += cstep; if (cc >= (unsigned)C) cc -= C;
        const int g = (int)fd_div(c0, fdCg);
        const float m = mrs[g * 4 + 0], r = mrs[g * 4 + 1];
        const float s1 = mrs[g * 4 + 2], s2 = mrs[g * 4 + 3];
        GNV8 xv, dv, out;
        xv.q = *reinterpret_cast<const uint4*>(x + base + i);
        dv.q = *reinterpret_cast<const uint4*>(dy + base + i);
        #pragma unroll
        for (int j = 0; j < 8; ++j) {
            const float xn = (bf2f(xv.u[j]) - m) * r;
            float dz = bf2f(dv.u[j]);
            if (SILU) {
                const float z = xn * gam[c0 + j] + bet[c0 + j];
                const float sig = 1.f / (1.f + __expf(-z));
                dz *= sig * (1.f + z * (1.f - sig));
            }
            out.u[j] = f2bf(r * (dz * gam[c0 + j] - (s1 + xn * s2) * inv_n));
        }
        *reinterpret_cast<uint4*>(dx + base + i) = out.q;
    }
}


std::vector<torch::Tensor> gn_silu_fwd(torch::Tensor x, torch::Tensor gamma,
                                       torch::Tensor beta, long groups,
                                       double eps, bool silu) {
    FD_FLUSH_STALE();
    TORCH_CHECK(x.is_cuda() && x.is_contiguous());
    const int B = x.size(0);
    const int C = x.size(-1);
    const long S = x.numel() / ((long)B * C);
    const int G = (int)groups;
    TORCH_CHECK(C % G == 0, "channels not divisible by groups");

    auto y = torch::empty_like(x);
    auto f32opt = x.options().dtype(at::kFloat);
    auto mean = torch::empty({(long)B * G}, f32opt);
    auto rstd = torch::empty({(long)B * G}, f32opt);
    auto gamma_f = gamma.to(at::kFloat).contiguous();
    auto beta_f = beta.to(at::kFloat).contiguous();
    auto stream = at::hip::getCurrentHIPStream();
    dim3 grid(B * G), block(256);

    const int Cg_f = C / G;
    #define LAUNCH_FWD(T, SILU_) \
        hipLaunchKernelGGL((gn_silu_fwd_kernel<T, SILU_>), grid, block, 0, stream, \
            (const T*)x.data_ptr(), gamma_f.data_ptr<float>(), beta_f.data_ptr<float>(), \
            (T*)y.data_ptr(), mean.data_ptr<float>(), rstd.data_ptr<float>(), \
            (int)S, C, G, (float)eps)
    if (x.scalar_type() == at::kBFloat16 && Cg_f % 8 == 0 && C <= 2048) {
        auto sums = torch::zeros({(long)B * 2 * G}, f32opt);
        const int chunk_rows = std::max(1, 32768 / C);
        dim3 g3(B, (S + chunk_rows - 1) / chunk_rows);
        const FastDiv fdCg = make_fastdiv(Cg_f);
        #define L_STATS(SILU_) hipLaunchKernelGGL((gn3_fwd_stats_kernel<SILU_>),             g3, dim3(GN3_NTH), 2 * G * sizeof(float), stream,             (const ushort*)x.data_ptr(), sums.data_ptr<float>(),             (int)S, C, G, Cg_f, chunk_rows, fdCg)
        #define L_APPLY(SILU_) hipLaunchKernelGGL((gn3_fwd_apply_kernel<SILU_>),             g3, dim3(GN3_NTH), (2 * G + 2 * C) * sizeof(float), stream,             (const ushort*)x.data_ptr(), sums.data_ptr<float>(),             gamma_f.data_ptr<float>(), beta_f.data_ptr<float>(),             (ushort*)y.data_ptr(), mean.data_ptr<float>(), rstd.data_ptr<float>(),             (int)S, C, G, Cg_f, chunk_rows, (float)eps, fdCg)
        if (silu) { L_STATS(true); L_APPLY(true); }
        else { L_STATS(false); L_APPLY(false); }
        #undef L_STATS
        #undef L_APPLY
    } else if (x.scalar_type() == at::kBFloat16) {
        if (silu) LAUNCH_FWD(ushort, true); else LAUNCH_FWD(ushort, false);
    } else {
        if (silu) LAUNCH_FWD(float, true); else LAUNCH_FWD(float, false);
    }
    #undef LAUNCH_FWD
    FD_CHECK_LAUNCH();
    return {y, mean, rstd};
}

std::vector<torch::Tensor> gn_silu_bwd(torch::Tensor dy, torch::Tensor x,
                                       torch::Tensor gamma, torch::Tensor beta,
                                       torch::Tensor mean, torch::Tensor rstd,
                                       long groups, bool silu,
                                       c10::optional<torch::Tensor> dgamma_sink,
                                       c10::optional<torch::Tensor> dbeta_sink) {
    FD_FLUSH_STALE();
    const int B = x.size(0);
    const int C = x.size(-1);
    const long S = x.numel() / ((long)B * C);
    const int G = (int)groups;
    const int Cg = C / G;
    TORCH_CHECK(Cg <= 256, "gn_silu_bwd: channels-per-group > 256 unsupported");

    const bool has_sink = dgamma_sink.has_value() && dgamma_sink->defined();
    TORCH_CHECK(has_sink == (dbeta_sink.has_value() && dbeta_sink->defined()),
                "gn_silu_bwd: pass both dgamma and dbeta sinks or neither");
    if (has_sink) {
        for (const torch::Tensor* t : {&*dgamma_sink, &*dbeta_sink})
            TORCH_CHECK(t->is_cuda() && t->device() == x.device() &&
                        t->is_contiguous() && t->scalar_type() == at::kFloat &&
                        t->numel() == C,
                        "gn_silu_bwd: sinks must be contiguous fp32 [C] tensors "
                        "on x's device");
    }

    auto dx = torch::empty_like(x);
    auto f32opt = x.options().dtype(at::kFloat);
    const long ngs = 2L * x.size(0) * G;
    auto zflat = torch::zeros({(has_sink ? 0L : 2L * C) + ngs}, f32opt);
    auto dgamma = has_sink ? *dgamma_sink : zflat.narrow(0, 0, C);
    auto dbeta = has_sink ? *dbeta_sink : zflat.narrow(0, C, C);
    auto gamma_f = gamma.to(at::kFloat).contiguous();
    auto beta_f = beta.to(at::kFloat).contiguous();
    auto stream = at::hip::getCurrentHIPStream();
    dim3 grid(B * G), block(256);
    const size_t smem = (2 * Cg + 4) * sizeof(float);

    #define LAUNCH_BWD(T, SILU_) \
        hipLaunchKernelGGL((gn_silu_bwd_kernel<T, SILU_>), grid, block, smem, stream, \
            (const T*)dy.data_ptr(), (const T*)x.data_ptr(), gamma_f.data_ptr<float>(), \
            beta_f.data_ptr<float>(), mean.data_ptr<float>(), rstd.data_ptr<float>(), \
            (T*)dx.data_ptr(), dgamma.data_ptr<float>(), dbeta.data_ptr<float>(), \
            (int)S, C, G)
    if (x.scalar_type() == at::kBFloat16 && Cg % 8 == 0 && C <= 2048) {
        auto gsums = zflat.narrow(0, has_sink ? 0L : 2L * C, ngs);
        static const long btarget = std::getenv("FD_GN_BLOCKS")
            ? atol(std::getenv("FD_GN_BLOCKS")) : 768L;
        const long bwant = std::max(1L, btarget / std::max(1, B));
        const int chunk_rows = std::max((int)((S + bwant - 1) / bwant),
                                        std::max(1, 32768 / C));
        dim3 g3(B, ((int)S + chunk_rows - 1) / chunk_rows);
        const FastDiv fdCg = make_fastdiv(Cg);
        #define L_BSTATS(SILU_) hipLaunchKernelGGL((gn3_bwd_stats_kernel<SILU_>),             g3, dim3(GN3_NTH), (4 * G + 4 * C) * sizeof(float), stream,             (const ushort*)dy.data_ptr(), (const ushort*)x.data_ptr(),             gamma_f.data_ptr<float>(), beta_f.data_ptr<float>(),             mean.data_ptr<float>(), rstd.data_ptr<float>(),             gsums.data_ptr<float>(), dgamma.data_ptr<float>(), dbeta.data_ptr<float>(),             (int)S, C, G, Cg, chunk_rows, fdCg)
        #define L_BAPPLY(SILU_) hipLaunchKernelGGL((gn3_bwd_apply_kernel<SILU_>),             g3, dim3(GN3_NTH), (4 * G + 2 * C) * sizeof(float), stream,             (const ushort*)dy.data_ptr(), (const ushort*)x.data_ptr(),             gamma_f.data_ptr<float>(), beta_f.data_ptr<float>(),             mean.data_ptr<float>(), rstd.data_ptr<float>(),             gsums.data_ptr<float>(), (ushort*)dx.data_ptr(),             (int)S, C, G, Cg, chunk_rows, fdCg)
        if (silu) { L_BSTATS(true); L_BAPPLY(true); }
        else { L_BSTATS(false); L_BAPPLY(false); }
        #undef L_BSTATS
        #undef L_BAPPLY
    } else if (x.scalar_type() == at::kBFloat16) {
        if (silu) LAUNCH_BWD(ushort, true); else LAUNCH_BWD(ushort, false);
    } else {
        if (silu) LAUNCH_BWD(float, true); else LAUNCH_BWD(float, false);
    }
    #undef LAUNCH_BWD
    FD_CHECK_LAUNCH();
    if (has_sink) return {dx};
    return {dx, dgamma.to(gamma.scalar_type()), dbeta.to(gamma.scalar_type())};
}
```

Measured before the change: 5344 images/s.

## Fuse residual-branch gradient add into GroupNorm backward; strided XCD-ordered attention kernels

GroupNorm gets a fork variant that returns the input as a second output, so the residual branch's gradient is summed inside the GN backward apply kernel instead of by a separate autograd accumulation. Attention forward and backward kernels now take per-tensor strides, so non-contiguous q/k/v/do views are no longer copied with .contiguous(). Blocks are also renumbered in an XCD-aware order so that heads of the same batch unit land together. These changes remove elementwise add and copy kernels and their memory traffic, at the cost of more index arithmetic and possibly less coalesced access for strided operands.

Result: faster. 5508 images/s, median of 6 (+3.1%).

```diff
diff --git a/flaxdiff_amd/models/common.py b/flaxdiff_amd/models/common.py
--- a/flaxdiff_amd/models/common.py
+++ b/flaxdiff_amd/models/common.py
@@ -89,6 +89,12 @@
         return ops.group_norm(x, self.num_groups, _cast(self.weight, x.dtype),
                               _cast(self.bias, x.dtype), self.eps, silu)
 
+    def forward_fork(self, x: torch.Tensor, silu: bool = False):
+        if x.is_cuda:
+            return ops.group_norm_fork(x, self.num_groups, self.weight,
+                                       self.bias, self.eps, silu)
+        return self.forward(x, silu), x
+
 
 class RMSNorm(nn.Module):
     def __init__(self, dim: int, eps: float = 1e-5):
@@ -310,8 +316,13 @@
 
     def forward(self, x: torch.Tensor, temb: torch.Tensor,
                 textemb: torch.Tensor = None, extra_features: torch.Tensor = None):
-        residual = x
-        out = self._norm_act(self.norm1, x)
+        if isinstance(self.norm1, GroupNorm):
+            out, residual = self.norm1.forward_fork(x, silu=self._fused_silu)
+            if not self._fused_silu:
+                out = self.activation(out)
+        else:
+            residual = x
+            out = self._norm_act(self.norm1, x)
         t = self.temb_projection(temb.to(out.dtype))
         if isinstance(self.conv1, Conv):
             out = self.conv1(out, badd=t)
diff --git a/flaxdiff_amd/ops/__init__.py b/flaxdiff_amd/ops/__init__.py
--- a/flaxdiff_amd/ops/__init__.py
+++ b/flaxdiff_amd/ops/__init__.py
@@ -118,6 +118,53 @@
     if _use_hip(x):
         return _GroupNormSiLUFn.apply(x.contiguous(), gamma, beta, groups, eps, silu)
     return reference.group_norm_nhwc(x, groups, gamma, beta, eps, silu)
+
+
+class _GroupNormForkFn(torch.autograd.Function):
+
+    @staticmethod
+    def forward(ctx, x, gamma, beta, groups, eps, silu):
+        ext = _require_ext()
+        ctx.set_materialize_grads(False)
+        y, mean, rstd = ext.gn_silu_fwd(x, gamma, beta, groups, eps, silu)
+        ctx.save_for_backward(x, gamma, mean, rstd)
+        ctx.groups = groups
+        ctx.silu = silu
+        ctx.beta = beta
+        ctx.gamma_param = gamma
+        return y, x
+
+    @staticmethod
+    def backward(ctx, dy, dx_pass):
+        x, gamma, mean, rstd = ctx.saved_tensors
+        ext = _require_ext()
+        if dy is None:
+            return dx_pass, None, None, None, None, None
+        add = None
+        if dx_pass is not None:
+            add = dx_pass.to(x.dtype).contiguous()
+        if ctx.needs_input_grad[1] and ctx.needs_input_grad[2]:
+            sg, sb = _grad_sink(ctx.gamma_param, "g"), _grad_sink(ctx.beta, "g")
+            if sg is not None and sb is not None:
+                (dx,) = ext.gn_silu_bwd(dy.contiguous(), x, gamma, ctx.beta,
+                                        mean, rstd, ctx.groups, ctx.silu,
+                                        sg, sb, add)
+                return dx, None, None, None, None, None
+        dx, dgamma, dbeta = ext.gn_silu_bwd(dy.contiguous(), x, gamma, ctx.beta,
+                                            mean, rstd, ctx.groups, ctx.silu,
+                                            None, None, add)
+        return dx, dgamma, dbeta, None, None, None
+
+
+def group_norm_fork_enabled() -> bool:
+    return os.environ.get("FD_GN_FORK_ADD", "1") != "0"
+
+
+def group_norm_fork(x: torch.Tensor, groups: int, gamma: torch.Tensor,
+                    beta: torch.Tensor, eps: float = 1e-5, silu: bool = False):
+    if _use_hip(x) and beta is not None and group_norm_fork_enabled():
+        return _GroupNormForkFn.apply(x.contiguous(), gamma, beta, groups, eps, silu)
+    return group_norm(x, groups, gamma, beta, eps, silu), x
 
 
 
@@ -594,6 +641,28 @@
 
 
 
+def _attn_view_ok(t: torch.Tensor) -> bool:
+    if t.dim() != 4:
+        return False
+    if t.is_contiguous():
+        return True
+    if t.stride(3) != 1 or t.data_ptr() % 16 or t.stride(2) >= 2 ** 31:
+        return False
+    return all(st > 0 and st % 8 == 0 for st in t.stride()[:3])
+
+
+def _attn_strided(q: torch.Tensor, k: torch.Tensor) -> bool:
+    if os.environ.get("FD_ATTN_STRIDED", "1") == "0":
+        return False
+    if os.environ.get("FD_ATTN_BWD_V1"):
+        return False
+    return k.shape[2] <= 128 and q.shape[3] <= 64
+
+
+def _attn_operand(t: torch.Tensor, strided: bool) -> torch.Tensor:
+    return t if strided and _attn_view_ok(t) else t.contiguous()
+
+
 class _AttentionFn(torch.autograd.Function):
     @staticmethod
     def forward(ctx, q, k, v, scale):
@@ -612,7 +681,8 @@
         if k.shape[2] <= 128 and q.shape[3] <= dmax:
             ext = _require_ext()
             fn = ext.attn_bwd_smallkv if use_v1 else ext.attn_bwd_smallkv_v2
-            dq, dk, dv = fn(q, k, v, do.contiguous(), lse, scale)
+            do = _attn_operand(do, not use_v1 and _attn_strided(q, k))
+            dq, dk, dv = fn(q, k, v, do, lse, scale)
             return dq, dk, dv, None
         qf, kf, vf, dof = q.float(), k.float(), v.float(), do.float()
         s = torch.einsum("bhqd,bhkd->bhqk", qf, kf) * scale
@@ -633,8 +703,10 @@
     if _use_hip(q):
         D = q.shape[-1]
         if D % 8 == 0 and D <= 128:
-            return _AttentionFn.apply(q.contiguous(), k.contiguous(),
-                                      v.contiguous(), scale)
+            strided = _attn_strided(q, k)
+            return _AttentionFn.apply(_attn_operand(q, strided),
+                                      _attn_operand(k, strided),
+                                      _attn_operand(v, strided), scale)
     return reference.attention(q, k, v, scale)
 
 
diff --git a/flaxdiff_amd/ops/hip/attention.hip b/flaxdiff_amd/ops/hip/attention.hip
--- a/flaxdiff_amd/ops/hip/attention.hip
+++ b/flaxdiff_amd/ops/hip/attention.hip
@@ -16,6 +16,9 @@
                      const ushort* __restrict__ V,
                      ushort* __restrict__ O,
                      float* __restrict__ LSE,
+                     const AttStrides qs, const AttStrides ks,
+                     const AttStrides vs, const AttStrides os,
+                     const int Bn, const int H, const int xcd_order,
                      const int Sq, const int Skv, const int D,
                      const float scale) {
     constexpr int Dp = NCH * 32;
@@ -28,17 +31,29 @@
     ushort* Vl = Kl + ATT_TILE * KROW;
     ushort* Pl = Vl + Dp * VROW;
 
-    const int bh = blockIdx.y;
-    const long q_blk = (long)blockIdx.x * (QI * 64);
+    const int ntile = (Sq + QI * 64 - 1) / (QI * 64);
+    int b, h, tile;
+    if (xcd_order) {
+        int unit;
+        if (!att_xcd_decode(blockIdx.x, H, Bn * ntile, unit, h)) return;
+        b = unit / ntile;
+        tile = unit - b * ntile;
+    } else {
+        const int bh = blockIdx.x / ntile;
+        tile = blockIdx.x - bh * ntile;
+        b = bh / H;
+        h = bh - b * H;
+    }
+    const long q_blk = (long)tile * (QI * 64);
     const int tid = threadIdx.x;
     const int lane = tid & 63;
     const int wid = tid >> 6;
     const int l15 = lane & 15;
     const int l4 = lane >> 4;
 
-    const ushort* Qb = Q + (long)bh * Sq * D;
-    const ushort* Kb = K + (long)bh * Skv * D;
-    const ushort* Vb = V + (long)bh * Skv * D;
+    const ushort* Qb = Q + (long)b * qs.b + (long)h * qs.h;
+    const ushort* Kb = K + (long)b * ks.b + (long)h * ks.h;
+    const ushort* Vb = V + (long)b * vs.b + (long)h * vs.h;
 
     ABF8 qf[QI][NCH];
     #pragma unroll
@@ -50,10 +65,10 @@
             const int d0 = c * 32 + l4 * 8;
             if (qrow < Sq && d0 < D) {
                 if (d0 + 8 <= D) {
-                    qf[qi][c].q = *reinterpret_cast<const uint4*>(Qb + qrow * D + d0);
+                    qf[qi][c].q = *reinterpret_cast<const uint4*>(Qb + qrow * qs.s + d0);
                 } else {
                     for (int j = 0; j < 8 && d0 + j < D; ++j)
-                        qf[qi][c].u[j] = Qb[qrow * D + d0 + j];
+                        qf[qi][c].u[j] = Qb[qrow * qs.s + d0 + j];
                 }
             }
         }
@@ -76,14 +91,15 @@
             ABF8 kval; kval.q = make_uint4(0, 0, 0, 0);
             ABF8 vval; vval.q = make_uint4(0, 0, 0, 0);
             if (kv0 + kv < Skv && d0 < D) {
-                const long src = (long)(kv0 + kv) * D + d0;
+                const long ksrc = (long)(kv0 + kv) * ks.s + d0;
+                const long vsrc = (long)(kv0 + kv) * vs.s + d0;
                 if (d0 + 8 <= D) {
-                    kval.q = *reinterpret_cast<const uint4*>(Kb + src);
-                    vval.q = *reinterpret_cast<const uint4*>(Vb + src);
+                    kval.q = *reinterpret_cast<const uint4*>(Kb + ksrc);
+                    vval.q = *reinterpret_cast<const uint4*>(Vb + vsrc);
                 } else {
                     for (int j = 0; j < 8 && d0 + j < D; ++j) {
-                        kval.u[j] = Kb[src + j];
-                        vval.u[j] = Vb[src + j];
+                        kval.u[j] = Kb[ksrc + j];
+                        vval.u[j] = Vb[vsrc + j];
                     }
                 }
             }
@@ -177,8 +193,8 @@
         }
     }
 
-    ushort* Ob = O + (long)bh * Sq * D;
-    float* Lb = LSE + (long)bh * Sq;
+    ushort* Ob = O + (long)b * os.b + (long)h * os.h;
+    float* Lb = LSE + ((long)b * H + h) * Sq;
     #pragma unroll
     for (int qi = 0; qi < QI; ++qi) {
         float inv_l[4];
@@ -194,7 +210,7 @@
             for (int r = 0; r < 4; ++r) {
                 const long qrow = qbase + l4 * 4 + r;
                 if (qrow < Sq)
-                    Ob[qrow * D + d] = f2bf(oacc[qi][f][r] * inv_l[r]);
+                    Ob[qrow * os.s + d] = f2bf(oacc[qi][f][r] * inv_l[r]);
             }
         }
         if (l15 == 0) {
@@ -211,13 +227,20 @@
 std::vector<torch::Tensor> attn_fwd(torch::Tensor q, torch::Tensor k,
                                     torch::Tensor v, double scale) {
     FD_FLUSH_STALE();
-    TORCH_CHECK(q.is_cuda() && q.is_contiguous() && q.dim() == 4);
-    TORCH_CHECK(q.scalar_type() == at::kBFloat16, "attn kernel is bf16");
+    TORCH_CHECK(q.is_cuda() && q.dim() == 4 && k.dim() == 4 && v.dim() == 4);
+    TORCH_CHECK(q.scalar_type() == at::kBFloat16 &&
+                k.scalar_type() == at::kBFloat16 &&
+                v.scalar_type() == at::kBFloat16, "attn kernel is bf16");
     const int B = q.size(0), H = q.size(1), Sq = q.size(2), D = q.size(3);
     const int Skv = k.size(2);
     TORCH_CHECK(D <= 128 && D % 8 == 0, "attn: D must be <=128, mult of 8; got ", D);
-
-    auto o = torch::empty_like(q);
+    TORCH_CHECK(k.size(0) == B && k.size(1) == H && k.size(3) == D &&
+                v.sizes() == k.sizes(), "attn: q/k/v shapes disagree");
+    TORCH_CHECK(att_layout_ok(q) && att_layout_ok(k) && att_layout_ok(v),
+                "attn: operands need a dense last dim, other strides multiples "
+                "of 8 elements and a 16-byte-aligned base, or to be dense");
+
+    auto o = torch::empty_strided(q.sizes(), q.strides(), q.options());
     auto lse = torch::empty({B, H, Sq}, q.options().dtype(at::kFloat));
 
     const int Dp = (D + 31) & ~31;
@@ -227,14 +250,23 @@
                          + (size_t)Dp * (ATT_TILE + 8)
                          + 4ul * 16 * (ATT_TILE + 8))
                         * sizeof(ushort);
-    dim3 grid((Sq + qi * 64 - 1) / (qi * 64), B * H);
+    const int ntile = (Sq + qi * 64 - 1) / (qi * 64);
+    const int xcd_order = (att_xcd_order_enabled() && H > 1 &&
+                           q.stride(1) < q.stride(2)) ? 1 : 0;
+    const long nblk = xcd_order
+        ? ((long)B * ntile + 7) / 8 * 8 * H : (long)B * H * ntile;
+    TORCH_CHECK(nblk < (1L << 31), "attn: grid too large");
+    dim3 grid((unsigned)nblk);
     auto stream = at::hip::getCurrentHIPStream();
     #define ATT_LAUNCH(QI_, NCH_) \
         hipLaunchKernelGGL((attn_fwd_kernel<QI_, NCH_>), grid, dim3(NTH), smem, \
                            stream, (const ushort*)q.data_ptr(), \
                            (const ushort*)k.data_ptr(), \
                            (const ushort*)v.data_ptr(), (ushort*)o.data_ptr(), \
-                           lse.data_ptr<float>(), Sq, Skv, D, (float)scale)
+                           lse.data_ptr<float>(), att_strides_of(q), \
+                           att_strides_of(k), att_strides_of(v), \
+                           att_strides_of(o), B, H, xcd_order, \
+                           Sq, Skv, D, (float)scale)
     if (nch == 1 && qi == 8) ATT_LAUNCH(8, 1);
     else if (nch == 1) ATT_LAUNCH(4, 1);
     else if (nch == 2) ATT_LAUNCH(2, 2);
diff --git a/flaxdiff_amd/ops/hip/attention_bwd_v2.hip b/flaxdiff_amd/ops/hip/attention_bwd_v2.hip
--- a/flaxdiff_amd/ops/hip/attention_bwd_v2.hip
+++ b/flaxdiff_amd/ops/hip/attention_bwd_v2.hip
@@ -28,6 +28,11 @@
                         ushort* __restrict__ dQ,
                         ushort* __restrict__ dKo,
                         ushort* __restrict__ dVo,
+                        const AttStrides qs, const AttStrides ks,
+                        const AttStrides vs, const AttStrides dos,
+                        const AttStrides dqst, const AttStrides dks,
+                        const AttStrides dvs,
+                        const int Bn, const int H, const int xcd_order,
                         const int Sq, const int Skv, const int D,
                         const float scale) {
     constexpr int NDP = DP / 16;
@@ -54,12 +59,21 @@
     ushort* Qp = dSt + 2 * PPS;
     ushort* dOp = Qp + NQI * PQS;
 
-    const int bh = blockIdx.x;
-    const ushort* Qb = Q + (long)bh * Sq * D;
-    const ushort* Kb = K + (long)bh * Skv * D;
-    const ushort* Vb = V + (long)bh * Skv * D;
-    const ushort* dOb = dO + (long)bh * Sq * D;
-    const float* lse_b = LSE + (long)bh * Sq;
+    int b, h;
+    if (xcd_order) {
+        if (!att_xcd_decode(blockIdx.x, H, Bn, b, h)) return;
+    } else {
+        b = blockIdx.x / H;
+        h = blockIdx.x - b * H;
+    }
+    const ushort* Qb = Q + (long)b * qs.b + (long)h * qs.h;
+    const ushort* Kb = K + (long)b * ks.b + (long)h * ks.h;
+    const ushort* Vb = V + (long)b * vs.b + (long)h * vs.h;
+    const ushort* dOb = dO + (long)b * dos.b + (long)h * dos.h;
+    ushort* dQb = dQ + (long)b * dqst.b + (long)h * dqst.h;
+    ushort* dKb = dKo + (long)b * dks.b + (long)h * dks.h;
+    ushort* dVb = dVo + (long)b * dvs.b + (long)h * dvs.h;
+    const float* lse_b = LSE + ((long)b * H + h) * Sq;
 
     for (int i = tid; i < NDP * PPS; i += NW * 64) {
         const int p = i / PPS;
@@ -67,8 +81,8 @@
         const int d = p * 16 + (i & 15);
         ushort kv = 0, vv = 0;
         if (j < Skv && d < D) {
-            kv = Kb[(long)j * D + d];
-            vv = Vb[(long)j * D + d];
+            kv = Kb[(long)j * ks.s + d];
+            vv = Vb[(long)j * vs.s + d];
         }
         Kp[i] = kv;
         Vp[i] = vv;
@@ -95,12 +109,12 @@
             const int d0 = c * 16 + half * 8;
             if (qvalid && qrow < Sq && d0 < D) {
                 if (d0 + 8 <= D) {
-                    qf[c].q = *reinterpret_cast<const uint4*>(Qb + qrow * D + d0);
-                    dof[c].q = *reinterpret_cast<const uint4*>(dOb + qrow * D + d0);
+                    qf[c].q = *reinterpret_cast<const uint4*>(Qb + qrow * qs.s + d0);
+                    dof[c].q = *reinterpret_cast<const uint4*>(dOb + qrow * dos.s + d0);
                 } else {
                     for (int t = 0; t < 8 && d0 + t < D; ++t) {
-                        qf[c].u[t] = Qb[qrow * D + d0 + t];
-                        dof[c].u[t] = dOb[qrow * D + d0 + t];
+                        qf[c].u[t] = Qb[qrow * qs.s + d0 + t];
+                        dof[c].u[t] = dOb[qrow * dos.s + d0 + t];
                     }
                 }
             }
@@ -272,10 +286,10 @@
                     for (int t = 0; t < 8; ++t)
                         outv.u[t] = (d0 + t < D) ? dqs[(d0 + t) * QROWS + qr] : (ushort)0;
                     if (d0 + 8 <= D) {
-                        *reinterpret_cast<uint4*>(dQ + ((long)bh * Sq + q0 + qr) * D + d0) = outv.q;
+                        *reinterpret_cast<uint4*>(dQb + (q0 + qr) * dqst.s + d0) = outv.q;
                     } else {
                         for (int t = 0; t < 8 && d0 + t < D; ++t)
-                            dQ[((long)bh * Sq + q0 + qr) * D + d0 + t] = outv.u[t];
+                            dQb[(q0 + qr) * dqst.s + d0 + t] = outv.u[t];
                     }
                 }
             }
@@ -308,8 +322,8 @@
     __syncthreads();
     for (int i = tid; i < Skv * D; i += NW * 64) {
         const int j = i / D, d = i - (i / D) * D;
-        dKo[((long)bh * Skv + j) * D + d] = f2bf(dkf[j * DP + d]);
-        dVo[((long)bh * Skv + j) * D + d] = f2bf(dvf[j * DP + d]);
+        dKb[(long)j * dks.s + d] = f2bf(dkf[j * DP + d]);
+        dVb[(long)j * dvs.s + d] = f2bf(dvf[j * DP + d]);
     }
 }
 
@@ -317,19 +331,33 @@
                                                torch::Tensor v, torch::Tensor dout,
                                                torch::Tensor lse, double scale) {
     FD_FLUSH_STALE();
-    TORCH_CHECK(q.is_cuda() && q.is_contiguous() && k.is_contiguous() &&
-                v.is_contiguous() && dout.is_contiguous());
-    TORCH_CHECK(q.scalar_type() == at::kBFloat16);
+    TORCH_CHECK(q.is_cuda() && q.dim() == 4);
+    TORCH_CHECK(q.scalar_type() == at::kBFloat16 &&
+                k.scalar_type() == at::kBFloat16 &&
+                v.scalar_type() == at::kBFloat16 &&
+                dout.scalar_type() == at::kBFloat16);
     const int B = q.size(0), H = q.size(1), Sq = q.size(2), D = q.size(3);
     const int Skv = k.size(2);
     TORCH_CHECK(Skv <= 128 && D <= 64);
+    TORCH_CHECK(k.dim() == 4 && k.size(0) == B && k.size(1) == H &&
+                k.size(3) == D && v.sizes() == k.sizes() &&
+                dout.sizes() == q.sizes() && lse.numel() == (long)B * H * Sq,
+                "attn_bwd_smallkv_v2: operand shapes disagree");
+    TORCH_CHECK(att_layout_ok(q) && att_layout_ok(k) && att_layout_ok(v) &&
+                att_layout_ok(dout),
+                "attn_bwd_smallkv_v2: operands need a dense last dim, other "
+                "strides multiples of 8 elements and a 16-byte-aligned base, or to be dense");
     auto lse_c = lse.contiguous();
     const int JT = ((Skv + 31) / 32) * 32;
     const int JTP = JT + 4;
 
-    auto dq = torch::empty_like(q);
-    auto dk = torch::empty_like(k);
-    auto dv = torch::empty_like(v);
+    auto dq = torch::empty_strided(q.sizes(), q.strides(), q.options());
+    auto dk = torch::empty_strided(k.sizes(), k.strides(), k.options());
+    auto dv = torch::empty_strided(v.sizes(), v.strides(), v.options());
+    const int xcd_order = (att_xcd_order_enabled() && H > 1 &&
+                           (q.stride(1) < q.stride(2) ||
+                            dout.stride(1) < dout.stride(2))) ? 1 : 0;
+    const int nblk = xcd_order ? (B + 7) / 8 * 8 * H : B * H;
 
     auto stream = at::hip::getCurrentHIPStream();
     const int nwaves = (JT / 32 == 4 || D > 32) ? 4 : 8;
@@ -348,11 +376,15 @@
                                 160 * 1024);
             attr_set[slot] = true;
         }
-        hipLaunchKernelGGL(kern, dim3(B * H), dim3(nwaves * 64), smem, stream,
+        hipLaunchKernelGGL(kern, dim3(nblk), dim3(nwaves * 64), smem, stream,
                            (const ushort*)q.data_ptr(), (const ushort*)k.data_ptr(),
                            (const ushort*)v.data_ptr(), (const ushort*)dout.data_ptr(),
                            lse_c.data_ptr<float>(), (ushort*)dq.data_ptr(),
                            (ushort*)dk.data_ptr(), (ushort*)dv.data_ptr(),
+                           att_strides_of(q), att_strides_of(k),
+                           att_strides_of(v), att_strides_of(dout),
+                           att_strides_of(dq), att_strides_of(dk),
+                           att_strides_of(dv), B, H, xcd_order,
                            Sq, Skv, D, (float)scale);
     };
     const int njf = JT / 32;
diff --git a/flaxdiff_amd/ops/hip/bindings.cpp b/flaxdiff_amd/ops/hip/bindings.cpp
--- a/flaxdiff_amd/ops/hip/bindings.cpp
+++ b/flaxdiff_amd/ops/hip/bindings.cpp
@@ -10,7 +10,8 @@
                                        torch::Tensor mean, torch::Tensor rstd,
                                        long groups, bool silu,
                                        c10::optional<torch::Tensor> dgamma_sink,
-                                       c10::optional<torch::Tensor> dbeta_sink);
+                                       c10::optional<torch::Tensor> dbeta_sink,
+                                       c10::optional<torch::Tensor> add);
 std::vector<torch::Tensor> rms_norm_fwd(torch::Tensor x, torch::Tensor gamma,
                                         double eps);
 std::vector<torch::Tensor> rms_norm_bwd(torch::Tensor dy, torch::Tensor x,
@@ -79,7 +80,8 @@
     m.def("gn_silu_bwd", &gn_silu_bwd, "fused GroupNorm+SiLU backward",
           py::arg("dy"), py::arg("x"), py::arg("gamma"), py::arg("beta"),
           py::arg("mean"), py::arg("rstd"), py::arg("groups"), py::arg("silu"),
-          py::arg("dgamma_sink") = py::none(), py::arg("dbeta_sink") = py::none());
+          py::arg("dgamma_sink") = py::none(), py::arg("dbeta_sink") = py::none(),
+          py::arg("add") = py::none());
     m.def("rms_norm_fwd", &rms_norm_fwd, "RMSNorm forward");
     m.def("rms_norm_bwd", &rms_norm_bwd, "RMSNorm backward",
           py::arg("dy"), py::arg("x"), py::arg("gamma"), py::arg("rrms"),
diff --git a/flaxdiff_amd/ops/hip/common.h b/flaxdiff_amd/ops/hip/common.h
--- a/flaxdiff_amd/ops/hip/common.h
+++ b/flaxdiff_amd/ops/hip/common.h
@@ -4,6 +4,7 @@
 #include <hip/hip_bf16.h>
 #include <hip/hip_fp16.h>
 #include <cstdint>
+#include <cstdlib>
 
 #define FD_WAVE 64
 
@@ -66,6 +67,41 @@
     return n - q * f.d;
 }
 
+struct AttStrides { long b, h; int s; };
+
+template <typename TensorT>
+inline AttStrides att_strides_of(const TensorT& t) {
+    return AttStrides{(long)t.stride(0), (long)t.stride(1), (int)t.stride(2)};
+}
+
+template <typename TensorT>
+inline bool att_layout_ok(const TensorT& t) {
+    if (t.dim() != 4) return false;
+    if (t.is_contiguous()) return true;
+    if (t.stride(2) >= (1L << 31)) return false;
+    if (t.stride(3) != 1) return false;
+    for (int i = 0; i < 3; ++i)
+        if (t.stride(i) <= 0 || t.stride(i) % 8 != 0) return false;
+    return reinterpret_cast<uintptr_t>(t.data_ptr()) % 16 == 0;
+}
+
+__device__ __forceinline__ bool att_xcd_decode(const int lin, const int H,
+                                               const int n_units,
+                                               int& unit, int& h) {
+    const int grp = lin / (8 * H), r = lin - grp * (8 * H);
+    h = r >> 3;
+    unit = grp * 8 + (r & 7);
+    return unit < n_units;
+}
+
+inline bool att_xcd_order_enabled() {
+    static const bool on = [] {
+        const char* e = std::getenv("FD_ATTN_XCD_ORDER");
+        return !(e && e[0] == '0');
+    }();
+    return on;
+}
+
 __device__ __forceinline__ float wave_reduce_sum(float v) {
     #pragma unroll
     for (int off = 32; off > 0; off >>= 1)
diff --git a/flaxdiff_amd/ops/hip/gn_silu.hip b/flaxdiff_amd/ops/hip/gn_silu.hip
--- a/flaxdiff_amd/ops/hip/gn_silu.hip
+++ b/flaxdiff_amd/ops/hip/gn_silu.hip
@@ -44,7 +44,7 @@
     }
 }
 
-template <typename T, bool SILU>
+template <typename T, bool SILU, bool HAS_ADD>
 __global__ void gn_silu_bwd_kernel(const T* __restrict__ dy,
                                    const T* __restrict__ x,
                                    const float* __restrict__ gamma,
@@ -54,6 +54,7 @@
                                    T* __restrict__ dx,
                                    float* __restrict__ dgamma,
                                    float* __restrict__ dbeta,
+                                   const T* __restrict__ add,
                                    int S, int C, int G) {
     const int b = blockIdx.x / G;
     const int g = blockIdx.x % G;
@@ -111,7 +112,9 @@
                 const float sig = 1.f / (1.f + expf(-z));
                 dz *= sig * (1.f + z * (1.f - sig));
             }
-            ElemIO<T>::st(dx + idx, rstd * (dz * gam - (s1 + xn * s2) * inv_n));
+            float dxv = rstd * (dz * gam - (s1 + xn * s2) * inv_n);
+            if (HAS_ADD) dxv += ElemIO<T>::ld(add + idx);
+            ElemIO<T>::st(dx + idx, dxv);
         }
         atomicAdd(dg_loc + c, dg_p);
         atomicAdd(db_loc + c, db_p);
@@ -302,7 +305,7 @@
     }
 }
 
-template <bool SILU>
+template <bool SILU, bool HAS_ADD>
 __global__ void gn3_bwd_apply_kernel(const ushort* __restrict__ dy,
                                      const ushort* __restrict__ x,
                                      const float* __restrict__ gamma,
@@ -310,6 +313,7 @@
                                      const float* __restrict__ mean_in,
                                      const float* __restrict__ rstd_in,
                                      const float* __restrict__ gsums,
+                                     const ushort* __restrict__ add,
                                      ushort* __restrict__ dx,
                                      const int S, const int C, const int G,
                                      const int Cg, const int chunk_rows,
@@ -344,9 +348,10 @@
         const int g = (int)fd_div(c0, fdCg);
         const float m = mrs[g * 4 + 0], r = mrs[g * 4 + 1];
         const float s1 = mrs[g * 4 + 2], s2 = mrs[g * 4 + 3];
-        GNV8 xv, dv, out;
+        GNV8 xv, dv, av, out;
         xv.q = *reinterpret_cast<const uint4*>(x + base + i);
         dv.q = *reinterpret_cast<const uint4*>(dy + base + i);
+        if (HAS_ADD) av.q = *reinterpret_cast<const uint4*>(add + base + i);
         #pragma unroll
         for (int j = 0; j < 8; ++j) {
             const float xn = (bf2f(xv.u[j]) - m) * r;
@@ -356,7 +361,9 @@
                 const float sig = 1.f / (1.f + __expf(-z));
                 dz *= sig * (1.f + z * (1.f - sig));
             }
-            out.u[j] = f2bf(r * (dz * gam[c0 + j] - (s1 + xn * s2) * inv_n));
+            float dxv = r * (dz * gam[c0 + j] - (s1 + xn * s2) * inv_n);
+            if (HAS_ADD) dxv += bf2f(av.u[j]);
+            out.u[j] = f2bf(dxv);
         }
         *reinterpret_cast<uint4*>(dx + base + i) = out.q;
     }
@@ -415,7 +422,8 @@
                                        torch::Tensor mean, torch::Tensor rstd,
                                        long groups, bool silu,
                                        c10::optional<torch::Tensor> dgamma_sink,
-                                       c10::optional<torch::Tensor> dbeta_sink) {
+                                       c10::optional<torch::Tensor> dbeta_sink,
+                                       c10::optional<torch::Tensor> add) {
     FD_FLUSH_STALE();
     const int B = x.size(0);
     const int C = x.size(-1);
@@ -435,6 +443,15 @@
                         "gn_silu_bwd: sinks must be contiguous fp32 [C] tensors "
                         "on x's device");
     }
+
+    const bool has_add = add.has_value() && add->defined();
+    if (has_add)
+        TORCH_CHECK(add->is_cuda() && add->device() == x.device() &&
+                    add->is_contiguous() && add->sizes() == x.sizes() &&
+                    add->scalar_type() == x.scalar_type(),
+                    "gn_silu_bwd: add must be a contiguous tensor of x's "
+                    "shape, dtype and device");
+    const void* add_p = has_add ? add->data_ptr() : nullptr;
 
     auto dx = torch::empty_like(x);
     auto f32opt = x.options().dtype(at::kFloat);
@@ -448,12 +465,15 @@
     dim3 grid(B * G), block(256);
     const size_t smem = (2 * Cg + 4) * sizeof(float);
 
-    #define LAUNCH_BWD(T, SILU_) \
-        hipLaunchKernelGGL((gn_silu_bwd_kernel<T, SILU_>), grid, block, smem, stream, \
+    #define LAUNCH_BWD_(T, SILU_, ADD_) \
+        hipLaunchKernelGGL((gn_silu_bwd_kernel<T, SILU_, ADD_>), grid, block, smem, stream, \
             (const T*)dy.data_ptr(), (const T*)x.data_ptr(), gamma_f.data_ptr<float>(), \
             beta_f.data_ptr<float>(), mean.data_ptr<float>(), rstd.data_ptr<float>(), \
             (T*)dx.data_ptr(), dgamma.data_ptr<float>(), dbeta.data_ptr<float>(), \
-            (int)S, C, G)
+            (const T*)add_p, (int)S, C, G)
+    #define LAUNCH_BWD(T, SILU_) \
+        do { if (has_add) LAUNCH_BWD_(T, SILU_, true); \
+             else LAUNCH_BWD_(T, SILU_, false); } while (0)
     if (x.scalar_type() == at::kBFloat16 && Cg % 8 == 0 && C <= 2048) {
         auto gsums = zflat.narrow(0, has_sink ? 0L : 2L * C, ngs);
         static const long btarget = std::getenv("FD_GN_BLOCKS")
@@ -464,9 +484,14 @@
         dim3 g3(B, ((int)S + chunk_rows - 1) / chunk_rows);
         const FastDiv fdCg = make_fastdiv(Cg);
         #define L_BSTATS(SILU_) hipLaunchKernelGGL((gn3_bwd_stats_kernel<SILU_>),             g3, dim3(GN3_NTH), (4 * G + 4 * C) * sizeof(float), stream,             (const ushort*)dy.data_ptr(), (const ushort*)x.data_ptr(),             gamma_f.data_ptr<float>(), beta_f.data_ptr<float>(),             mean.data_ptr<float>(), rstd.data_ptr<float>(),             gsums.data_ptr<float>(), dgamma.data_ptr<float>(), dbeta.data_ptr<float>(),             (int)S, C, G, Cg, chunk_rows, fdCg)
-        #define L_BAPPLY(SILU_) hipLaunchKernelGGL((gn3_bwd_apply_kernel<SILU_>),             g3, dim3(GN3_NTH), (4 * G + 2 * C) * sizeof(float), stream,             (const ushort*)dy.data_ptr(), (const ushort*)x.data_ptr(),             gamma_f.data_ptr<float>(), beta_f.data_ptr<float>(),             mean.data_ptr<float>(), rstd.data_ptr<float>(),             gsums.data_ptr<float>(), (ushort*)dx.data_ptr(),             (int)S, C, G, Cg, chunk_rows, fdCg)
-        if (silu) { L_BSTATS(true); L_BAPPLY(true); }
-        else { L_BSTATS(false); L_BAPPLY(false); }
+        #define L_BAPPLY(SILU_, ADD_) hipLaunchKernelGGL((gn3_bwd_apply_kernel<SILU_, ADD_>),             g3, dim3(GN3_NTH), (4 * G + 2 * C) * sizeof(float), stream,             (const ushort*)dy.data_ptr(), (const ushort*)x.data_ptr(),             gamma_f.data_ptr<float>(), beta_f.data_ptr<float>(),             mean.data_ptr<float>(), rstd.data_ptr<float>(),             gsums.data_ptr<float>(), (const ushort*)add_p, (ushort*)dx.data_ptr(),             (int)S, C, G, Cg, chunk_rows, fdCg)
+        if (silu) {
+            L_BSTATS(true);
+            if (has_add) L_BAPPLY(true, true); else L_BAPPLY(true, false);
+        } else {
+            L_BSTATS(false);
+            if (has_add) L_BAPPLY(false, true); else L_BAPPLY(false, false);
+        }
         #undef L_BSTATS
         #undef L_BAPPLY
     } else if (x.scalar_type() == at::kBFloat16) {
@@ -475,6 +500,7 @@
         if (silu) LAUNCH_BWD(float, true); else LAUNCH_BWD(float, false);
     }
     #undef LAUNCH_BWD
+    #undef LAUNCH_BWD_
     FD_CHECK_LAUNCH();
     if (has_sink) return {dx};
     return {dx, dgamma.to(gamma.scalar_type()), dbeta.to(gamma.scalar_type())};
```
